# ViTAE-Transformer/MTP

Measured on AMD Instinct MI355X. Metric: images/sec pretrain step (ViT-L+RVSA, 224^2, bf16), higher is better.
Workload: dtype bf16; 1 GPU; ViT-L + RVSA backbone fwd+bwd + grad all-reduce + clip + AdamW, 224x224, batch 64 per GPU (BASELINE configs[2]/[3]); global_batch=64, parallelism=dp1, activation_checkpointing=False, heads=sum_i mean(f_i)

## Files before the change

### include/mtp_hip.h

```cpp
#ifndef MTP_HIP_H_
#define MTP_HIP_H_

#include <stddef.h>
#include <stdint.h>

#ifdef __cplusplus
extern "C" {
#endif

typedef void* mtp_stream_t;

typedef enum { MTP_F32 = 0, MTP_BF16 = 1, MTP_F64 = 2  } mtp_dtype;

enum { MTP_OK = 0, MTP_ERR_ARG = -1, MTP_ERR_UNSUPPORTED = -2 };

typedef enum {
    MTP_EPI_BIAS = 0,
    MTP_EPI_BIAS_GELU = 1,
    MTP_EPI_BIAS_RES = 2,
    MTP_EPI_DGELU = 3,
    MTP_EPI_BIAS_GELU_DG = 4,
    MTP_EPI_MUL = 5
} mtp_epilogue;

// ... 54 lines not shown

int mtp_gemm_nt(const mtp_gemm_args* args, mtp_stream_t stream);
typedef enum {
    MTP_GEMM_NT_FAMILY_SB = 0,
    MTP_GEMM_NT_FAMILY_SB8 = 1,
    MTP_GEMM_NT_FAMILY_REG = 2,
    MTP_GEMM_NT_FAMILY_P8 = 3,
    MTP_GEMM_NT_FAMILY_STRIP = 4
} mtp_gemm_nt_family;
struct mtp_gemm_nt_plan {
    int family;
    int tile_m;
    int order;
    int persistent;
    int store_policy;
};
int mtp_gemm_nt_plan(const mtp_gemm_args* args, int cus, struct mtp_gemm_nt_plan* out);
int mtp_gemm_nt_tile(const mtp_gemm_args* args);
int64_t mtp_gemm_nt_workspace_bytes(void);
int mtp_gemm_tn(const mtp_gemm_args* args, mtp_stream_t stream);
#define MTP_MAX_GROUPED_GEMMS 32
int mtp_gemm_tn_grouped(const mtp_gemm_args* args, int count, mtp_stream_t stream);
int mtp_sum_partials_batch(const float* const* parts, float* const* outs, const int64_t* numel, const int* splits, int count,
                           mtp_stream_t stream);

int mtp_layernorm_fwd(const void* x, int x_dtype, const float* gamma, const float* beta, void* y, int y_dtype,
                      float* mean, float* rstd, int64_t rows, int64_t C, float eps, int fuse_gelu, mtp_stream_t stream);
int64_t mtp_layernorm_bwd_partial_rows(int64_t rows);
int mtp_layernorm_bwd(const void* dy, int dy_dtype, const void* x, int x_dtype, const float* mean, const float* rstd,
                      const float* gamma, const float* beta, int fuse_gelu,
                      const float* dres, const float* extra, void* dx, int dx_dtype,
                      void* dx_copy, int copy_dtype, const float* copy_scale, int64_t rows_per_sample,
                      float* dgamma_part, float* dbeta_part, int64_t part_ld, int64_t rows, int64_t C, mtp_stream_t stream);
int mtp_layernorm_bwd_win(const void* dy, int dy_dtype, const void* x, int x_dtype, const float* mean, const float* rstd,
                          const float* gamma, const float* dres, const float* extra, void* dx, int dx_dtype,
                          void* dx_copy, int copy_dtype, const float* copy_scale, int64_t rows_per_sample,
                          float* dgamma_part, float* dbeta_part, int64_t part_ld, int64_t rows, int64_t C,
                          const float* win_add, int64_t B, int64_t Hp, int64_t Wp, mtp_stream_t stream);
int mtp_layernorm_residual_fwd(const void* h, int dtype, const float* gamma, const float* beta, const float* x, const float* layer_scale,
                               const float* sample_scale, int64_t rows_per_sample, float* out, void* out_act, float* mean, float* rstd,
                               int64_t rows, int64_t C, float eps, mtp_stream_t stream);
int mtp_layernorm_residual_bwd(const float* dout, const void* h, int dtype, const float* mean, const float* rstd, const float* gamma, const float* beta,
                               const float* layer_scale, const float* sample_scale, int64_t rows_per_sample, void* dh, float* part,
                               int64_t rows, int64_t C, mtp_stream_t stream);
int mtp_reduce_rows_f32(const float* part, int64_t ld, float* out, int64_t rows, int64_t C, int accumulate, mtp_stream_t stream);
#define MTP_REDUCE_BATCH_MAX 32
int mtp_reduce_rows_batched_f32(const float* const* parts, float* const* outs, int n, int64_t ld, int64_t rows, int64_t C, int accumulate,
                                mtp_stream_t stream);
int mtp_reduce_rows_t_f32(const float* part, int64_t ld, float* out, int64_t rows, int64_t R, int64_t C, int accumulate, mtp_stream_t stream);
int mtp_reduce_rows_t_batched_f32(const float* const* parts, float* const* outs, int n, int64_t ld, int64_t rows, int64_t R, int64_t C, int accumulate,
                                  mtp_stream_t stream);
int mtp_colsum(const void* dY, int dtype, int64_t ld, float* out, int64_t M, int64_t N, mtp_stream_t stream);
int mtp_colsum_acc(const void* dY, int dtype, int64_t ld, float* out, int64_t M, int64_t N, mtp_stream_t stream);

int mtp_patchify(const float* img, void* cols, int dtype, int64_t B, int64_t Cin, int64_t H, int64_t W, int64_t P, mtp_stream_t stream);
int mtp_unpatchify(const void* cols, int dtype, float* dimg, int64_t B, int64_t Cin, int64_t H, int64_t W, int64_t P, mtp_stream_t stream);
int mtp_preprocess_patchify(const uint8_t* img, void* cols, int dtype, int64_t B, int64_t H, int64_t W, int64_t P, int64_t pad_divisor,
                            const float* mean, const float* std, int bgr_to_rgb, float pad_value, mtp_stream_t stream);
int mtp_cast(const void* src, int src_dtype, void* dst, int dst_dtype, int64_t n, mtp_stream_t stream);
int mtp_transpose_cast(const float* src, void* dst, int dst_dtype, int64_t R, int64_t C, mtp_stream_t stream);
typedef struct {
    const float* src;
    void* w;
    void* wt;
    int64_t R, C;
    int64_t tile0;
    int32_t f32_out;
    float wd;
} mtp_wimg_desc;
int mtp_weight_images(const mtp_wimg_desc* descs_dev, int n, int64_t total_tiles, int act_dtype, mtp_stream_t stream);
int mtp_adamw_weight_images(const mtp_wimg_desc* descs_dev, int n, int64_t total_tiles, int act_dtype, float* p_base, const float* g_base, float* m_base, float* v_base,
                            const float* hyper, const float* sqnorm, float max_norm, float grad_scale, mtp_stream_t stream);
int mtp_adamw_weight_images_lr(const mtp_wimg_desc* descs_dev, const float* desc_lr, int n, int64_t total_tiles, int act_dtype, float* p_base, const float* g_base,
                               float* m_base, float* v_base, const float* hyper, const float* sqnorm, float max_norm, float grad_scale, mtp_stream_t stream);
int mtp_convt_pack(const float* w, void* wg, void* wgT, int dtype, int64_t Cin, int64_t Cout, mtp_stream_t stream);
int mtp_convt_unpack_grad(const float* dwg, float* dw, int64_t Cin, int64_t Cout, mtp_stream_t stream);
int mtp_tokens_to_nchw(const void* x, int x_dtype, void* out, int out_dtype, int64_t B, int64_t Hp, int64_t Wp, int64_t C, int levels, mtp_stream_t stream);
int mtp_nchw_to_tokens(const void* f, int f_dtype, void* out, int out_dtype, int64_t B, int64_t Hp, int64_t Wp, int64_t C, int levels, mtp_stream_t stream);
int mtp_maxpool2_tokens_fwd(const float* x, void* y, int y_dtype, int64_t B, int64_t Hp, int64_t Wp, int64_t C, mtp_stream_t stream);
int mtp_maxpool2_tokens_bwd(const float* x, const void* dy, int dy_dtype, float* dx, int accumulate, int64_t B, int64_t Hp, int64_t Wp, int64_t C, mtp_stream_t stream);
int mtp_axpy_f32(float* y, const float* x, float alpha, int64_t n, mtp_stream_t stream);
#define MTP_MAX_SEGMENTS 12
int mtp_copy_segments_f32(const float* const* src, float* const* dst, const int64_t* count, int n, mtp_stream_t stream);
int mtp_scale_rows_cast(const float* src, void* dst, int dst_dtype, const float* scale, int64_t rows_per_sample, int64_t rows, int64_t C, mtp_stream_t stream);

int mtp_im2col3x3(const void* x, int x_dtype, int64_t sN, int64_t sH, int64_t sW, int64_t sC, void* cols, int cols_dtype,
                  int64_t N, int64_t H, int64_t W, int64_t Cin, int64_t stride, int64_t Kp, mtp_stream_t stream);
int mtp_col2im3x3(const void* dcols, int cols_dtype, float* dx, int64_t sN, int64_t sH, int64_t sW, int64_t sC,
                  int64_t N, int64_t H, int64_t W, int64_t Cin, int64_t stride, int64_t Kp, int accumulate, mtp_stream_t stream);
int mtp_conv3x3_pack(const float* w, void* w2, void* w2t, int dtype, int64_t Cout, int64_t Cin, int64_t Kp, mtp_stream_t stream);
int mtp_conv3x3_unpack_grad(const float* dw2, float* dw, int64_t Cout, int64_t Cin, int64_t Kp, mtp_stream_t stream);
int mtp_pack_rows_padded(const float* w, void* wp, void* wpt, int dtype, int64_t R, int64_t C, int64_t Rp, mtp_stream_t stream);
int mtp_cast_pad_rows(const float* src, int64_t n, void* dst, int dst_dtype, int64_t ld, int64_t rows, mtp_stream_t stream);
int mtp_copy_rows(const void* src, int64_t src_ld, void* dst, int64_t dst_ld, int dtype, int64_t n, int64_t rows, mtp_stream_t stream);
int mtp_dwconv3x3_fwd(const void* x, const float* w, const float* bias, void* y, int dtype, int64_t N, int64_t H, int64_t W, int64_t C, mtp_stream_t stream);
int mtp_dwconv3x3_bwd_dx(const void* dy, int dtype, const float* w, float* dx, int accumulate, int64_t N, int64_t H, int64_t W, int64_t C, mtp_stream_t stream);
int64_t mtp_dwconv3x3_bwd_dw_partial_rows(int64_t N, int64_t H, int64_t W);
int mtp_dwconv3x3_bwd_dw(const void* dy, const void* x, int dtype, float* part, int64_t N, int64_t H, int64_t W, int64_t C, mtp_stream_t stream);
typedef enum { MTP_CONV_OP_IM2COL3X3 = 0, MTP_CONV_OP_COL2IM3X3 = 1, MTP_CONV_OP_DWCONV3X3_FWD = 2, MTP_CONV_OP_DWCONV3X3_BWD_DX = 3, MTP_CONV_OP_DWCONV3X3_BWD_DW = 4 } mtp_conv_op;
typedef enum {
    MTP_CONV_KERNEL_NONE = 0,
    MTP_CONV_KERNEL_ELEMENT = 1,
    MTP_CONV_KERNEL_V8 = 2,
    MTP_CONV_KERNEL_P8 = 3,
    MTP_CONV_KERNEL_PX4 = 4
} mtp_conv_kernel_family;
int mtp_conv_kernel(int op, const void* src, int src_dtype, int64_t sN, int64_t sH, int64_t sW, int64_t sC, const void* dst, int dst_dtype,
                    const float* w, const float* bias, int64_t N, int64_t H, int64_t W, int64_t C, int64_t stride, int64_t Kp);
int mtp_dwconv_fwd(const void* x, const float* w, const float* bias, void* y, int dtype, int64_t N, int64_t H, int64_t W, int64_t C, int k, mtp_stream_t stream);
int mtp_dwconv_bwd_dx(const void* dy, int dtype, const float* w, float* dx, int accumulate, int64_t N, int64_t H, int64_t W, int64_t C, int k, mtp_stream_t stream);
int mtp_dwconv_bwd_dw(const void* dy, const void* x, int dtype, float* dw, float* db, int64_t N, int64_t H, int64_t W, int64_t C, int k, mtp_stream_t stream);
// ... 24 lines not shown
    MTP_FULL_BWD_V3 = 1,
    MTP_FULL_BWD_FLASH = 3,
    MTP_FULL_BWD_THREE_PASS = 4,
    MTP_FULL_BWD_SINGLE_WG = 5,
    MTP_RVSA_FWD_GENERIC = 1,
    MTP_RVSA_FWD_MFMA = 2,
    MTP_RVSA_BWD_GENERIC = 1,
    MTP_RVSA_BWD_MFMA_DENSE = 2,
    MTP_RVSA_BWD_MFMA_ATOMIC = 3
};
int mtp_full_attn_kernel(int dtype, int64_t Hp, int64_t Wp, int backward);
int mtp_rvsa_attn_kernel(int dtype, int64_t Hp, int64_t Wp, int64_t heads, int backward);

int mtp_rvsa_pool_fwd(const void* x, int dtype, float* avg, float* pooled, int64_t B, int64_t Hp, int64_t Wp, int64_t C, mtp_stream_t stream);
int mtp_rvsa_pool_bwd(const float* dpooled, const float* avg, void* dx, int dtype, int accumulate, int64_t B, int64_t Hp, int64_t Wp, int64_t C, mtp_stream_t stream);
int mtp_rvsa_sampling_fwd(const void* x, int dtype, const float* w, const float* bias, float* avg, float* pooled, float* samp,
                          int64_t B, int64_t Hp, int64_t Wp, int64_t C, int64_t N, mtp_stream_t stream);
int mtp_rvsa_sampling_bwd(const float* dsamp, const float* w, const float* avg, void* dx, int dtype,
                          int64_t B, int64_t Hp, int64_t Wp, int64_t C, int64_t N, mtp_stream_t stream);
int mtp_rvsa_sampling_bwd_win(const float* dsamp, const float* w, const float* avg, float* g, int64_t windows, int64_t C, int64_t N, mtp_stream_t stream);
int mtp_small_linear_fwd(const float* x, const float* w, const float* b, float* y, int64_t R, int64_t N, int64_t K, mtp_stream_t stream);
int mtp_small_linear_bwd(const float* x, const float* w, const float* dy, float* dx, float* dw, float* db, int64_t R, int64_t N, int64_t K, mtp_stream_t stream);
int mtp_small_linear_dw_segments(const float* x, const float* dy, int64_t R, int64_t N, int64_t K, int nseg, const int64_t* seg_rows,
                                 float* const* dw, float* const* db, mtp_stream_t stream);
int mtp_small_linear_dw_segments_batched(const float* const* xs, const float* const* dys, int count, int64_t R, int64_t N, int64_t K, int nseg,
                                         const int64_t* seg_rows, float* const* dw, float* const* db, mtp_stream_t stream);
int mtp_rvsa_attn_fwd(const void* qkv, const float* samp, void* o, float* lse, int dtype,
                      const float* rel_h, const float* rel_w, const float* bias_table,
                      int64_t B, int64_t Hp, int64_t Wp, int64_t heads, int64_t hd, float scale, mtp_stream_t stream);
int mtp_rvsa_attn_bwd(const void* qkv, const float* samp, const void* o, const void* dout, const float* lse,
                      void* dqkv, float* dkv_f32, float* dsamp, float* rel_part, float* tab_part, int dtype,
                      const float* rel_h, const float* rel_w, const float* bias_table,
                      int64_t B, int64_t Hp, int64_t Wp, int64_t heads, int64_t hd, float scale, mtp_stream_t stream);

int mtp_zero_segments_f32(float* base, const int64_t* start, const int64_t* count, int n, mtp_stream_t stream);
int mtp_sqnorm_f32(const float* g, float* out, int64_t n, mtp_stream_t stream);
int mtp_sqnorm_segments_f32(const float* base, const int64_t* start, const int64_t* count, int n, float* out, mtp_stream_t stream);
int mtp_adamw_flat(float* p, const float* g, float* m, float* v, int64_t n, const int64_t* seg_start, const float* seg_wd, int nseg,
                   const float* hyper, const float* sqnorm, float max_norm, float grad_scale, mtp_stream_t stream);
int mtp_adamw_flat_lr(float* p, const float* g, float* m, float* v, int64_t n, const int64_t* seg_start, const float* seg_wd, const float* seg_lr, int nseg,
                      const float* hyper, const float* sqnorm, float max_norm, float grad_scale, mtp_stream_t stream);

typedef struct {
    int64_t N, H, W;
    int kernel_h, kernel_w, stride_h, stride_w, pad_h, pad_w, dilation_h, dilation_w;
    int group, group_channels;
    float offset_scale;
    int im2col_step;
    int remove_center;
    int variant;
} mtp_dcnv3_geom;
int mtp_dcnv3_out_size(const mtp_dcnv3_geom* geom, int64_t* Ho, int64_t* Wo);
int mtp_dcnv3_fwd(const void* input, const void* offset, const void* mask, void* output, int dtype, const mtp_dcnv3_geom* geom, mtp_stream_t stream);
int mtp_dcnv3_bwd(const void* input, const void* offset, const void* mask, const void* grad_output, int dtype, float* grad_input, float* grad_offset,
                  float* grad_mask, const mtp_dcnv3_geom* geom, mtp_stream_t stream);
int mtp_dcnv3_bwd_act(const void* input, const void* offset, const void* mask, const void* grad_output, int dtype, float* grad_input, float* grad_offset,
                      float* grad_mask, void* grad_offset_act, int64_t act_ld, const mtp_dcnv3_geom* geom, mtp_stream_t stream);

typedef enum {
    MTP_DCNV3_KERNEL_NONE = 0,
    MTP_DCNV3_FWD9 = 1,
    MTP_DCNV3_FWD_VEC8 = 2,
    MTP_DCNV3_FWD_SCALAR = 3,
    MTP_DCNV3_F64 = 4,
    MTP_DCNV3_BWD_WINDOW_R2 = 5,
    MTP_DCNV3_BWD_WINDOW_R3 = 6,
// ... 96 lines not shown
```

### mtp_amd/_lib.py

```python
import ctypes as C
import os

_HERE = os.path.dirname(os.path.abspath(__file__))
LIB_PATH = os.environ.get("MTP_HIP_LIB") or os.path.join(_HERE, "libmtp_hip.so")

MTP_F32, MTP_BF16, MTP_F64 = 0, 1, 2
EPI_BIAS, EPI_BIAS_GELU, EPI_BIAS_RES, EPI_DGELU, EPI_BIAS_GELU_DG, EPI_MUL = 0, 1, 2, 3, 4, 5

GEMM_NT_REG_STAGED = 1
GEMM_ORDER_SHIFT, GEMM_ORDER_PLAIN, GEMM_ORDER_GROUPED, GEMM_ORDER_ROW_MAJOR, GEMM_ORDER_MASK = 1, 1 << 1, 2 << 1, 3 << 1, 3 << 1
GEMM_TNG_PLAIN_ORDER = 1 << 1
GEMM_TN_REG_TRANSPOSE = 1 << 4
GEMM_NT_SB8, GEMM_NT_NO_SB8 = 1 << 5, 1 << 6
GEMM_NT_P8, GEMM_NT_P8_224, GEMM_NT_P8_256, GEMM_NT_P8_MASK, GEMM_NT_NO_P8 = 1 << 8, 2 << 8, 3 << 8, 3 << 8, 1 << 10
GEMM_NT_PERSIST, GEMM_TN_TR_FULL_ONLY, GEMM_NT_NO_PERSIST = 1 << 15, 1 << 15, 1 << 16
GEMM_NT_STRIP, GEMM_NT_NO_STRIP = 1 << 17, 1 << 18
GEMM_TNG_PLAIN_PHASES = 1 << 19
GEMM_STORE_SHIFT, GEMM_STORE_NT, GEMM_STORE_SC1, GEMM_STORE_PLAIN, GEMM_STORE_MASK = 20, 1 << 20, 2 << 20, 3 << 20, 3 << 20
GEMM_NT_FAMILY_SB, GEMM_NT_FAMILY_SB8, GEMM_NT_FAMILY_REG, GEMM_NT_FAMILY_P8, GEMM_NT_FAMILY_STRIP = 0, 1, 2, 3, 4

CONV_OP_IM2COL3X3, CONV_OP_COL2IM3X3, CONV_OP_DWCONV3X3_FWD, CONV_OP_DWCONV3X3_BWD_DX, CONV_OP_DWCONV3X3_BWD_DW = 0, 1, 2, 3, 4
CONV_KERNEL_NONE, CONV_KERNEL_ELEMENT, CONV_KERNEL_V8, CONV_KERNEL_P8, CONV_KERNEL_PX4 = 0, 1, 2, 3, 4
DCNV3_KERNEL_NONE, DCNV3_FWD9, DCNV3_FWD_VEC8, DCNV3_FWD_SCALAR, DCNV3_F64 = 0, 1, 2, 3, 4
DCNV3_BWD_WINDOW_R2, DCNV3_BWD_WINDOW_R3, DCNV3_BWD_3X3_OS1, DCNV3_BWD_3X3_OS2, DCNV3_BWD_SCATTER_SHFL, DCNV3_BWD_SCATTER_ATOMIC = 5, 6, 7, 8, 9, 10
# ... 23 lines not shown
class WimgDesc(C.Structure):
    _fields_ = [("src", p), ("w", p), ("wt", p), ("R", i64), ("C", i64), ("tile0", i64), ("f32_out", C.c_int32), ("wd", C.c_float)]


class Dcnv3Geom(C.Structure):
    _fields_ = [("N", i64), ("H", i64), ("W", i64), ("kernel_h", C.c_int32), ("kernel_w", C.c_int32), ("stride_h", C.c_int32), ("stride_w", C.c_int32),
                ("pad_h", C.c_int32), ("pad_w", C.c_int32), ("dilation_h", C.c_int32), ("dilation_w", C.c_int32), ("group", C.c_int32),
                ("group_channels", C.c_int32), ("offset_scale", C.c_float), ("im2col_step", C.c_int32), ("remove_center", C.c_int32), ("variant", C.c_int32)]


SIGNATURES = {
    "mtp_weight_images": (i32, [p, i32, i64, i32, p]),
    "mtp_dwconv_fwd": (i32, [p, p, p, p, i32, i64, i64, i64, i64, i32, p]),
    "mtp_dwconv_bwd_dx": (i32, [p, i32, p, p, i32, i64, i64, i64, i64, i32, p]),
    "mtp_dwconv_bwd_dw": (i32, [p, p, i32, p, p, i64, i64, i64, i64, i32, p]),
    "mtp_center_feature_scale_fwd": (i32, [p, p, p, i64, p, i32, i64, i64, i64, p]),
    "mtp_center_feature_scale_bwd": (i32, [p, p, p, p, i64, p, p, p, i32, i64, i64, i64, p]),
    "mtp_dcnv3_out_size": (i32, [C.POINTER(Dcnv3Geom), C.POINTER(i64), C.POINTER(i64)]),
    "mtp_dcnv3_fwd": (i32, [p, p, p, p, i32, C.POINTER(Dcnv3Geom), p]),
    "mtp_dcnv3_bwd": (i32, [p, p, p, p, i32, p, p, p, C.POINTER(Dcnv3Geom), p]),
    "mtp_dcnv3_bwd_act": (i32, [p, p, p, p, i32, p, p, p, p, i64, C.POINTER(Dcnv3Geom), p]),
    "mtp_dcnv3_kernel": (i32, [p, p, p, p, p, p, p, i32, C.POINTER(Dcnv3Geom), i32]),
    "mtp_conv_kernel": (i32, [i32, p, i32, i64, i64, i64, i64, p, i32, p, p, i64, i64, i64, i64, i64, i64]),
    "mtp_gemm_nt": (i32, [C.POINTER(GemmArgs), p]),
    "mtp_gemm_nt_plan": (i32, [C.POINTER(GemmArgs), i32, C.POINTER(GemmNtPlan)]),
    "mtp_gemm_nt_tile": (i32, [C.POINTER(GemmArgs)]),
    "mtp_gemm_nt_workspace_bytes": (i64, []),
    "mtp_gemm_tn": (i32, [C.POINTER(GemmArgs), p]),
    "mtp_gemm_tn_grouped": (i32, [C.POINTER(GemmArgs), i32, p]),
    "mtp_sum_partials_batch": (i32, [p, p, p, p, i32, p]),
    "mtp_layernorm_fwd": (i32, [p, i32, p, p, p, i32, p, p, i64, i64, f32, i32, p]),
    "mtp_layernorm_bwd_partial_rows": (i64, [i64]),
    "mtp_layernorm_bwd": (i32, [p, i32, p, i32, p, p, p, p, i32, p, p, p, i32, p, i32, p, i64, p, p, i64, i64, i64, p]),
    "mtp_reduce_rows_f32": (i32, [p, i64, p, i64, i64, i32, p]),
    "mtp_reduce_rows_batched_f32": (i32, [p, p, i32, i64, i64, i64, i32, p]),
    "mtp_reduce_rows_t_f32": (i32, [p, i64, p, i64, i64, i64, i32, p]),
    "mtp_reduce_rows_t_batched_f32": (i32, [p, p, i32, i64, i64, i64, i64, i32, p]),
    "mtp_copy_segments_f32": (i32, [p, p, p, i32, p]),
    "mtp_colsum": (i32, [p, i32, i64, p, i64, i64, p]),
    "mtp_colsum_acc": (i32, [p, i32, i64, p, i64, i64, p]),
    "mtp_patchify": (i32, [p, p, i32, i64, i64, i64, i64, i64, p]),
    "mtp_preprocess_patchify": (i32, [p, p, i32, i64, i64, i64, i64, i64, C.POINTER(f32), C.POINTER(f32), i32, f32, p]),
    "mtp_unpatchify": (i32, [p, i32, p, i64, i64, i64, i64, i64, p]),
    "mtp_cast": (i32, [p, i32, p, i32, i64, p]),
    "mtp_transpose_cast": (i32, [p, p, i32, i64, i64, p]),
    "mtp_convt_pack": (i32, [p, p, p, i32, i64, i64, p]),
    "mtp_convt_unpack_grad": (i32, [p, p, i64, i64, p]),
    "mtp_tokens_to_nchw": (i32, [p, i32, p, i32, i64, i64, i64, i64, i32, p]),
    "mtp_nchw_to_tokens": (i32, [p, i32, p, i32, i64, i64, i64, i64, i32, p]),
    "mtp_maxpool2_tokens_fwd": (i32, [p, p, i32, i64, i64, i64, i64, p]),
    "mtp_maxpool2_tokens_bwd": (i32, [p, p, i32, p, i32, i64, i64, i64, i64, p]),
    "mtp_axpy_f32": (i32, [p, p, f32, i64, p]),
    "mtp_scale_rows_cast": (i32, [p, p, i32, p, i64, i64, i64, p]),
    "mtp_im2col3x3": (i32, [p, i32, i64, i64, i64, i64, p, i32, i64, i64, i64, i64, i64, i64, p]),
    "mtp_col2im3x3": (i32, [p, i32, p, i64, i64, i64, i64, i64, i64, i64, i64, i64, i64, i32, p]),
    "mtp_conv3x3_pack": (i32, [p, p, p, i32, i64, i64, i64, p]),
    "mtp_conv3x3_unpack_grad": (i32, [p, p, i64, i64, i64, p]),
    "mtp_pack_rows_padded": (i32, [p, p, p, i32, i64, i64, i64, p]),
    "mtp_cast_pad_rows": (i32, [p, i64, p, i32, i64, i64, p]),
    "mtp_copy_rows": (i32, [p, i64, p, i64, i32, i64, i64, p]),
    "mtp_dwconv3x3_fwd": (i32, [p, p, p, p, i32, i64, i64, i64, i64, p]),
    "mtp_dwconv3x3_bwd_dx": (i32, [p, i32, p, p, i32, i64, i64, i64, i64, p]),
    "mtp_dwconv3x3_bwd_dw_partial_rows": (i64, [i64, i64, i64]),
    "mtp_dwconv3x3_bwd_dw": (i32, [p, p, i32, p, i64, i64, i64, i64, p]),
    "mtp_softmax_groups_fwd": (i32, [p, i64, p, i32, i64, i64, i64, p]),
    "mtp_softmax_groups_bwd": (i32, [p, p, p, i64, i32, i64, i64, i64, p]),
    "mtp_scale_residual_fwd": (i32, [p, p, i32, p, p, i64, p, p, i64, i64, p]),
    "mtp_scale_residual_bwd_partial_rows": (i64, [i64]),
    "mtp_scale_residual_bwd": (i32, [p, p, i32, p, p, i64, p, p, i64, i64, p]),
    "mtp_comm_unique_id": (i32, [p]),
    "mtp_comm_init": (i32, [p, i32, i32, C.POINTER(C.c_void_p)]),
    "mtp_comm_allreduce_bucket": (i32, [p, p, i64, p]),
    "mtp_comm_allreduce_bucket_dt": (i32, [p, p, i64, i32, p]),
    "mtp_comm_reduce_scatter_bucket": (i32, [p, p, i64, i32, i32, p]),
    "mtp_comm_allgather_bucket": (i32, [p, p, i64, i32, i32, p]),
    "mtp_comm_info": (i32, [p, p]),
    "mtp_comm_destroy": (i32, [p]),
    "mtp_full_attn_fwd": (i32, [p, p, p, i32, p, p, i64, i64, i64, i64, i64, f32, p]),
    "mtp_full_attn_bwd_workspace_floats": (i64, [i64, i64, i64, i64]),
    "mtp_full_attn_bwd": (i32, [p, p, p, p, p, i32, p, p, p, p, i64, i64, i64, i64, i64, f32, p]),
    "mtp_full_attn_kernel": (i32, [i32, i64, i64, i32]),
    "mtp_rvsa_attn_kernel": (i32, [i32, i64, i64, i64, i32]),
    "mtp_rvsa_pool_fwd": (i32, [p, i32, p, p, i64, i64, i64, i64, p]),
    "mtp_rvsa_pool_bwd": (i32, [p, p, p, i32, i32, i64, i64, i64, i64, p]),
    "mtp_rvsa_sampling_fwd": (i32, [p, i32, p, p, p, p, p, i64, i64, i64, i64, i64, p]),
    "mtp_rvsa_sampling_bwd": (i32, [p, p, p, p, i32, i64, i64, i64, i64, i64, p]),
    "mtp_rvsa_sampling_bwd_win": (i32, [p, p, p, p, i64, i64, i64, p]),
    "mtp_layernorm_residual_fwd": (i32, [p, i32, p, p, p, p, p, i64, p, p, p, p, i64, i64, f32, p]),
    "mtp_layernorm_residual_bwd": (i32, [p, p, i32, p, p, p, p, p, p, i64, p, p, i64, i64, p]),
    "mtp_layernorm_bwd_win": (i32, [p, i32, p, i32, p, p, p, p, p, p, i32, p, i32, p, i64, p, p, i64, i64, i64, p, i64, i64, i64, p]),
    "mtp_small_linear_fwd": (i32, [p, p, p, p, i64, i64, i64, p]),
    "mtp_small_linear_bwd": (i32, [p, p, p, p, p, p, i64, i64, i64, p]),
    "mtp_small_linear_dw_segments": (i32, [p, p, i64, i64, i64, i32, p, p, p, p]),
    "mtp_small_linear_dw_segments_batched": (i32, [p, p, i32, i64, i64, i64, i32, p, p, p, p]),
    "mtp_rvsa_attn_fwd": (i32, [p, p, p, p, i32, p, p, p, i64, i64, i64, i64, i64, f32, p]),
    "mtp_rvsa_attn_bwd": (i32, [p, p, p, p, p, p, p, p, p, p, i32, p, p, p, i64, i64, i64, i64, i64, f32, p]),
    "mtp_zero_segments_f32": (i32, [p, p, p, i32, p]),
    "mtp_sqnorm_f32": (i32, [p, p, i64, p]),
    "mtp_sqnorm_segments_f32": (i32, [p, p, p, i32, p, p]),
    "mtp_adamw_flat": (i32, [p, p, p, p, i64, p, p, i32, p, p, f32, f32, p]),
    "mtp_adamw_weight_images": (i32, [p, i32, i64, i32, p, p, p, p, p, p, f32, f32, p]),
    "mtp_adamw_flat_lr": (i32, [p, p, p, p, i64, p, p, p, i32, p, p, f32, f32, p]),
    "mtp_adamw_weight_images_lr": (i32, [p, p, i32, i64, i32, p, p, p, p, p, p, f32, f32, p]),
    "mtp_bn_partial_rows": (i64, [i64]),
    "mtp_bn_stats": (i32, [p, i32, i64, p, p, p, i64, i64, p]),
    "mtp_bn_finalize": (i32, [p, p, C.c_double, p, p, f32, f32, p, p, i64, p]),
    "mtp_bn_apply": (i32, [p, i32, i64, p, p, p, p, i32, p, i32, i64, i64, i64, p]),
    "mtp_bn_bwd_stats": (i32, [p, i32, i64, p, i32, i64, p, p, p, p, i32, p, p, i64, i64, p]),
    "mtp_bn_bwd_dx": (i32, [p, i32, i64, p, i32, i64, p, p, p, p, i32, p, C.c_double, p, i32, i64, i64, i64, p]),
    "mtp_resize_bilinear_fwd": (i32, [p, i32, i64, p, i32, i64, i64, i64, i64, i64, i64, i64, i32, p]),
    "mtp_resize_bilinear_bwd": (i32, [p, i32, i64, p, i64, i64, i64, i64, i64, i64, i64, i32, p]),
    "mtp_adaptive_avg_pool_fwd": (i32, [p, i32, i64, p, i32, i64, i64, i64, i64, i64, p]),
    "mtp_adaptive_avg_pool_bwd": (i32, [p, i32, p, i64, i64, i64, i64, i64, i64, i32, p]),
    "mtp_channel_scale": (i32, [p, i32, i64, p, i64, p, i32, i64, i64, i64, p]),
    "mtp_seg_ce_workspace_bytes": (i64, [i64, i64, i64, i64]),
    "mtp_seg_ce": (i32, [p, i32, i64, i64, i64, i64, i64, p, i32, i64, i64, i32, f32, p, p, i64, p, i64, p]),
    "mtp_seg_window_accumulate": (i32, [p, i32, i64, i64, i64, i64, i64, p, i64, i64, i64, i64, i64, i64, i64, p]),
    "mtp_seg_argmax_areas": (i32, [p, i64, i64, i64, i64, i64, p, p, i32, p, p, p, i32, i32, p, p]),
    "mtp_seg_areas": (i32, [p, i32, p, i32, i64, i64, i32, p, p]),
    "mtp_fuse_pair_fwd": (i32, [p, i32, p, i32, i64, i64, i64, i64, i64, i32, p]),
    "mtp_fuse_pair_bwd": (i32, [p, i64, p, i32, p, i64, i64, i64, i64, i32, p]),
    "mtp_unet_up_cat_fwd": (i32, [p, i64, i64, p, i64, i64, i32, p, i32, i64, i64, i64, i64, i64, i64, p]),
    "mtp_unet_up_cat_bwd": (i32, [p, i64, p, i64, i64, p, i64, i64, i64, i64, i64, i64, i64, i32, p]),
    "mtp_gap_fwd": (i32, [p, i32, p, i64, i64, i64, p]),
    "mtp_gap_bwd": (i32, [p, p, i32, i64, i64, i64, p]),
    "mtp_cls_ce": (i32, [p, p, p, p, f32, p, p, p, p, p, p, p, i64, i64, i64, p]),
    "mtp_cls_head_bwd": (i32, [p, p, p, p, p, p, i64, i64, i64, i32, p]),
    "mtp_cls_hits": (i32, [p, p, i64, i64, C.POINTER(C.c_int32), i32, f32, i32, p, p]),
    "mtp_box_iou": (i32, [p, p, p, i64, i64, i32, i32, i32, f32, p]),
# ... 41 lines not shown
```

### mtp_amd/csrc/attn.hip

```cpp
#include <stdlib.h>

#include "attn_launch.h"
#include "attn_rvsa_common.h"

namespace {

constexpr int KT = 32;

template <typename T>
__device__ __forceinline__ void load_row(const T* p, float (&r)[HD], float mul = 1.0f) {
#pragma unroll
    for (int i = 0; i < HD / 8; ++i) {
        float t[8];
        load8(p + 8 * i, t);
#pragma unroll
        for (int e = 0; e < 8; ++e) r[8 * i + e] = t[e] * mul;
    }
}
template <typename T>
__device__ __forceinline__ void store_row(T* p, const float (&r)[HD], float mul = 1.0f) {
#pragma unroll
    for (int i = 0; i < HD / 8; ++i) {
        float t[8];
#pragma unroll
// ... 799 lines not shown
                               (const float*)workspace, N, (int)Hp, (int)Wp, (int)heads, scale);
        }
        return mtp_launch_status();
    }
    const size_t lds = full_bwd1_lds(Hp, Wp);
    dim3 grid((unsigned)(B * heads)), block(256);
    hipStream_t s = (hipStream_t)stream;
    if (dtype == MTP_BF16) {
        (void)hipFuncSetAttribute((const void*)full_attn_bwd_kernel<bf16_t>, hipFuncAttributeMaxDynamicSharedMemorySize, (int)lds);
        hipLaunchKernelGGL((full_attn_bwd_kernel<bf16_t>), grid, block, lds, s, (const bf16_t*)qkv, (const bf16_t*)o, (const bf16_t*)dout, lse, (bf16_t*)dqkv,
                           rel_h, rel_w, drel_part, N, (int)Hp, (int)Wp, (int)heads, scale);
    } else {
        (void)hipFuncSetAttribute((const void*)full_attn_bwd_kernel<float>, hipFuncAttributeMaxDynamicSharedMemorySize, (int)lds);
        hipLaunchKernelGGL((full_attn_bwd_kernel<float>), grid, block, lds, s, (const float*)qkv, (const float*)o, (const float*)dout, lse, (float*)dqkv,
                           rel_h, rel_w, drel_part, N, (int)Hp, (int)Wp, (int)heads, scale);
    }
    return mtp_launch_status();
}

extern "C" int mtp_rvsa_attn_fwd(const void* qkv, const float* samp, void* o, float* lse, int dtype,
                                 const float* rel_h, const float* rel_w, const float* bias_table,
                                 int64_t B, int64_t Hp, int64_t Wp, int64_t heads, int64_t hd, float scale, mtp_stream_t stream) {
    if (!qkv || !samp || !o || !lse || !rel_h || !rel_w || !bias_table || B <= 0 || Hp < 7 || Wp < 7 || heads <= 0) return MTP_ERR_ARG;
    if (hd != HD) return MTP_ERR_UNSUPPORTED;
    const RvsaGeom g = make_geom(Hp, Wp, heads);
    dim3 grid((unsigned)(B * g.nh * g.nw * heads)), block(64);
    hipStream_t s = (hipStream_t)stream;
    if (rvsa_fwd_family(dtype) == MTP_RVSA_FWD_MFMA)
        return mtp_rvsa_fwd_mfma_launch(qkv, samp, o, lse, rel_h, rel_w, bias_table, B, Hp, Wp, heads, scale, s);
    hipLaunchKernelGGL(rvsa_attn_fwd_kernel, grid, block, 0, s, (const float*)qkv, samp, (float*)o, lse, rel_h, rel_w, bias_table, g, scale);
    return mtp_launch_status();
}

extern "C" int mtp_rvsa_attn_bwd(const void* qkv, const float* samp, const void* o, const void* dout, const float* lse,
                                 void* dqkv, float* dkv_f32, float* dsamp, float* rel_part, float* tab_part, int dtype,
                                 const float* rel_h, const float* rel_w, const float* bias_table,
                                 int64_t B, int64_t Hp, int64_t Wp, int64_t heads, int64_t hd, float scale, mtp_stream_t stream) {
    if (!qkv || !samp || !o || !dout || !lse || !dqkv || !dkv_f32 || !dsamp || !rel_part || !tab_part || !rel_h || !rel_w || !bias_table) return MTP_ERR_ARG;
    if (B <= 0 || Hp < 7 || Wp < 7 || heads <= 0) return MTP_ERR_ARG;
    if (hd != HD) return MTP_ERR_UNSUPPORTED;
    const RvsaGeom g = make_geom(Hp, Wp, heads);
    const int64_t Ttok = B * Hp * Wp, C = heads * HD;
    hipStream_t s = (hipStream_t)stream;
    const int family = rvsa_bwd_family(dtype, Hp, Wp, heads);
    if (family == MTP_RVSA_BWD_MFMA_DENSE)
        return mtp_rvsa_bwd_mfma_launch(qkv, samp, o, dout, lse, dqkv, dkv_f32, dsamp, rel_part, tab_part, rel_h, rel_w, bias_table, B, Hp, Wp, heads, scale, s);
    hipError_t e = hipMemsetAsync(dkv_f32, 0, sizeof(float) * (size_t)(Ttok * 2 * C), s);
    if (e != hipSuccess) return (int)e;
    dim3 grid((unsigned)(B * g.nh * g.nw * heads)), block(64);
    int64_t cb = (Ttok * 2 * C / 4 + 255) / 256;
    dim3 cgrid((unsigned)(cb > 8192 ? 8192 : cb)), cblock(256);
    if (family == MTP_RVSA_BWD_MFMA_ATOMIC) {
        const int rc = mtp_rvsa_bwd_mfma_launch(qkv, samp, o, dout, lse, dqkv, dkv_f32, dsamp, rel_part, tab_part, rel_h, rel_w, bias_table, B, Hp, Wp, heads, scale, s);
        if (rc) return rc;
        hipLaunchKernelGGL((dkv_convert_kernel<bf16_t>), cgrid, cblock, 0, s, dkv_f32, (bf16_t*)dqkv, Ttok, (int)C);
    } else {
        hipLaunchKernelGGL(rvsa_attn_bwd_kernel, grid, block, 0, s, (const float*)qkv, samp, (const float*)o, (const float*)dout, lse, (float*)dqkv,
                           dkv_f32, dsamp, rel_part, tab_part, rel_h, rel_w, bias_table, g, scale);
        hipLaunchKernelGGL((dkv_convert_kernel<float>), cgrid, cblock, 0, s, dkv_f32, (float*)dqkv, Ttok, (int)C);
    }
    return mtp_launch_status();
}
```

### mtp_amd/csrc/attn_launch.h

```cpp
#pragma once
#include <hip/hip_runtime.h>
#include <stdint.h>

int mtp_rvsa_fwd_mfma_launch(const void* qkv, const float* samp, void* o, float* lse, const float* rel_h, const float* rel_w, const float* bias_table,
                             int64_t B, int64_t Hp, int64_t Wp, int64_t heads, float scale, hipStream_t s);
int mtp_rvsa_bwd_mfma_launch(const void* qkv, const float* samp, const void* o, const void* dout, const float* lse, void* dqkv, float* dkv, float* dsamp,
                             float* rel_part, float* tab_part, const float* rel_h, const float* rel_w, const float* bias_table,
                             int64_t B, int64_t Hp, int64_t Wp, int64_t heads, float scale, hipStream_t s);
int mtp_rvsa_bwd_mfma_scatter_mode(int64_t Hp, int64_t Wp, int64_t heads);
bool mtp_full_v3_fits(int64_t Hp, int64_t Wp);
int mtp_full_fwd_flash_keys(int64_t Hp, int64_t Wp);
bool mtp_full_bwd_flash_fits(int64_t Hp, int64_t Wp);
int mtp_full_v3_fwd_launch(const void* qkv, void* o, float* lse, const float* rel_h, const float* rel_w, int64_t B, int64_t Hp, int64_t Wp, int64_t heads,
                           float scale, hipStream_t s);
int mtp_full_v3_bwd_launch(const void* qkv, const void* o, const void* dout, const float* lse, void* dqkv, const float* rel_h, const float* rel_w,
                           float* drel_part, int64_t B, int64_t Hp, int64_t Wp, int64_t heads, float scale, hipStream_t s);
int mtp_full_fwd_flash_launch(const void* qkv, void* o, float* lse, const float* rel_h, const float* rel_w, int64_t B, int64_t Hp, int64_t Wp, int64_t heads,
                              float scale, hipStream_t s);
int mtp_full_bwd_flash_launch(const void* qkv, const void* o, const void* dout, const float* lse, void* dqkv, const float* rel_h, const float* rel_w,
                              float* drel_part, float* workspace, int64_t B, int64_t Hp, int64_t Wp, int64_t heads, float scale, hipStream_t s);
```

### mtp_amd/csrc/attn_rvsa_bwd4.hip

```cpp
#include <stdlib.h>

#include "attn_launch.h"
#include "attn_rvsa_common.h"

namespace {

typedef __attribute__((ext_vector_type(2))) __bf16 bf16x2v_t;
constexpr int TP = 136;
constexpr int SMP_F = 18;

__global__ __launch_bounds__(256, 3) void rvsa_bwd5_mfma_kernel(const bf16_t* __restrict__ qkv, const float* __restrict__ samp, const bf16_t* __restrict__ o, const bf16_t* __restrict__ dout,
                                                            const float* __restrict__ lse, bf16_t* __restrict__ dqkv, float* __restrict__ dkv, float* __restrict__ dsamp,
                                                            float* __restrict__ rel_part, float* __restrict__ tab_part,
                                                            const float* __restrict__ rel_h, const float* __restrict__ rel_w, const float* __restrict__ bias_table,
                                                            RvsaGeom g, float scale) {
    __shared__ __attribute__((aligned(16))) char Ks[64 * 128];
    __shared__ __attribute__((aligned(16))) char Vs[64 * 128];
    __shared__ __attribute__((aligned(16))) char R2[2 * 64 * 128];
    __shared__ float QR[26 * 64];
    constexpr int DQP = 65;
    __shared__ float dQR[26 * DQP];
    __shared__ float tab[176];
    __shared__ float lses[64];
    __shared__ float delta[64];
// ... 784 lines not shown
#pragma unroll
            for (int kk = 0; kk < 2; ++kk) {
                float w[8];
#pragma unroll
                for (int e = 0; e < 8; ++e)
                    w[e] = live * fmaxf(0.f, 1.f - fabsf(kx[8 * kk + e] - X)) * fmaxf(0.f, 1.f - fabsf(ky[8 * kk + e] - Y));
                af[kk] = pack_bf16x8(w[0], w[1], w[2], w[3], w[4], w[5], w[6], w[7]);
            }
#pragma unroll
            for (int dt = 0; dt < 4; ++dt) {
                f32x4_t ak = {0.f, 0.f, 0.f, 0.f}, av = {0.f, 0.f, 0.f, 0.f};
#pragma unroll
                for (int kk = 0; kk < 2; ++kk) {
                    ak = mma(af[kk], bk[dt][kk], ak);
                    av = mma(af[kk], bv[dt][kk], av);
                }
#pragma unroll
                for (int r = 0; r < 4; ++r) {
                    const int t2 = 16 * ti + 4 * gq + r;
                    if (t2 < N) {
                        float* drow = dkv + ((int64_t)b * N + t2) * (2 * C) + h * HD + 16 * dt + fr;
                        if (ak[r] != 0.f) atomicAdd(drow, ak[r]);
                        if (av[r] != 0.f) atomicAdd(drow + C, av[r]);
                    }
                }
            }
        }
    }
}

constexpr int SCB = 224;

__global__ __launch_bounds__(256, 2) void rvsa_scatter_gemm_kernel(const bf16_t* __restrict__ dsel, const float* __restrict__ samp, bf16_t* __restrict__ dqkv,
                                                                  RvsaGeom g) {
    __shared__ __attribute__((aligned(16))) char Kimg[SCB * 128];
    __shared__ __attribute__((aligned(16))) char Vimg[SCB * 128];
    __shared__ __attribute__((aligned(16))) float xs[SCB];
    __shared__ __attribute__((aligned(16))) float ys[SCB];
    const int tid = threadIdx.x, lane = tid & 63, wave = tid >> 6, fr = lane & 15, gq = lane >> 4;
    const int H = g.heads, nW = g.nh * g.nw, S = nW * 49;
    const int h = blockIdx.x % H, b = blockIdx.x / H;
    const int C = H * HD, N = g.Hp * g.Wp;
    const int t0 = blockIdx.y * SCB, nt = (N - t0) < SCB ? (N - t0) : SCB;
    const int64_t ld = 3 * (int64_t)C;
    float X[4], Y[4], live[4];
    f32x4_t dk[4][4], dv[4][4];
#pragma unroll
    for (int i = 0; i < 4; ++i) {
        const int tl = 16 * (wave + 4 * i) + fr;
        const int tc = t0 + (tl < nt ? tl : nt - 1);
        const int ty = tc / g.Wp, tx = tc - ty * g.Wp;
        X[i] = (float)(tx + g.pad_l);
        Y[i] = (float)(ty + g.pad_t);
        live[i] = tl < nt ? 1.f : 0.f;
#pragma unroll
        for (int dt = 0; dt < 4; ++dt) {
            dk[i][dt] = f32x4_t{0.f, 0.f, 0.f, 0.f};
            dv[i][dt] = f32x4_t{0.f, 0.f, 0.f, 0.f};
        }
    }
    const int ntile = (nt + 15) / 16;
    const float ylo = (float)(t0 / g.Wp + g.pad_t) - 1.0f, yhi = (float)((t0 + nt - 1) / g.Wp + g.pad_t) + 1.0f;
    for (int c0 = 0; c0 < S; c0 += SCB) {
        __syncthreads();
        int hit = 0;
        if (tid < SCB) {
            const int sg = c0 + tid;
            float x = -1.0e4f, y = -1.0e4f;
            if (sg < S) {
                const int w = sg / 49, k = sg - 49 * w;
                const Sample sa = make_sample<true>(g, samp + (int64_t)(b * nW + w) * 5 * H, h, w / g.nw, w % g.nw, k / 7, k % 7);
                x = (float)sa.x0 + sa.fx;
                y = (float)sa.y0 + sa.fy;
            }
// ... 57 lines not shown
#pragma unroll
    for (int i = 0; i < 4; ++i) {
        const int tl = 16 * (wave + 4 * i) + fr;
        if (tl < nt) {
#pragma unroll
            for (int dt = 0; dt < 4; ++dt) {
                const int o = tl * 128 + (((2 * dt + (gq >> 1)) ^ (tl & 7)) << 4) + (gq & 1) * 8;
                *reinterpret_cast<uint2*>(Kimg + o) = make_uint2(pack_bf16x2(dk[i][dt][0], dk[i][dt][1]), pack_bf16x2(dk[i][dt][2], dk[i][dt][3]));
                *reinterpret_cast<uint2*>(Vimg + o) = make_uint2(pack_bf16x2(dv[i][dt][0], dv[i][dt][1]), pack_bf16x2(dv[i][dt][2], dv[i][dt][3]));
            }
        }
    }
    __syncthreads();
    for (int idx = tid; idx < nt * 16; idx += 256) {
        const int tl = idx >> 4, m = (idx >> 3) & 1, ch = idx & 7;
        const uint4 v = *reinterpret_cast<const uint4*>((m ? Vimg : Kimg) + swz(tl, ch));
        *reinterpret_cast<uint4*>(dqkv + ((int64_t)b * N + t0 + tl) * ld + (1 + m) * C + h * HD + 8 * ch) = v;
    }
}

}

int mtp_rvsa_bwd_mfma_scatter_mode(int64_t Hp, int64_t Wp, int64_t heads) {
    static const bool dense = []() { const char* e = getenv("MTP_RVSA_SCATTER"); return e && e[0] == 'd'; }();
    if (dense) return 1;
    const RvsaGeom g = make_geom(Hp, Wp, heads);
    const int64_t N = Hp * Wp, nW = (int64_t)g.nh * g.nw;
    const bool fits = Hp <= 64 && Wp <= 64 && nW * (2 * 49 * HD * 2) <= N * 2 * HD * 4;
    return fits ? 4 : 1;
}

int mtp_rvsa_bwd_mfma_launch(const void* qkv, const float* samp, const void* o, const void* dout, const float* lse, void* dqkv, float* dkv, float* dsamp,
                             float* rel_part, float* tab_part, const float* rel_h, const float* rel_w, const float* bias_table,
                             int64_t B, int64_t Hp, int64_t Wp, int64_t heads, float scale, hipStream_t s) {
    const RvsaGeom g = make_geom(Hp, Wp, heads);
    const int mode = mtp_rvsa_bwd_mfma_scatter_mode(Hp, Wp, heads);
    const dim3 grid((unsigned)(B * g.nh * g.nw * heads));
    if (mode == 4) {
        static const bool old4 = []() { const char* e = getenv("MTP_RVSA_BWD"); return e && e[0] == '4'; }();
        if (old4)
            hipLaunchKernelGGL(rvsa_bwd4_mfma_kernel<4>, grid, dim3(256), 0, s, (const bf16_t*)qkv, samp, (const bf16_t*)o, (const bf16_t*)dout, lse,
                               (bf16_t*)dqkv, dkv, dsamp, rel_part, tab_part, rel_h, rel_w, bias_table, g, scale);
        else
            hipLaunchKernelGGL(rvsa_bwd5_mfma_kernel, grid, dim3(256), 0, s, (const bf16_t*)qkv, samp, (const bf16_t*)o, (const bf16_t*)dout, lse,
                               (bf16_t*)dqkv, dkv, dsamp, rel_part, tab_part, rel_h, rel_w, bias_table, g, scale);
        const int64_t N = Hp * Wp;
        hipLaunchKernelGGL(rvsa_scatter_gemm_kernel, dim3((unsigned)(B * heads), (unsigned)((N + SCB - 1) / SCB)), dim3(256), 0, s, (const bf16_t*)dkv, samp, (bf16_t*)dqkv, g);
    } else {
        hipLaunchKernelGGL(rvsa_bwd4_mfma_kernel<1>, grid, dim3(256), 0, s, (const bf16_t*)qkv, samp, (const bf16_t*)o, (const bf16_t*)dout, lse,
                           (bf16_t*)dqkv, dkv, dsamp, rel_part, tab_part, rel_h, rel_w, bias_table, g, scale);
    }
    return mtp_launch_status();
}
```

### mtp_amd/csrc/common.h

```cpp
#pragma once
#include <hip/hip_runtime.h>
#include <stdint.h>

#include "../../include/mtp_hip.h"

#define MTP_WAVE 64

typedef __attribute__((ext_vector_type(8))) __bf16 bf16x8_t;
typedef __attribute__((ext_vector_type(4))) float f32x4_t;

struct bf16_t {
    uint16_t bits;
};

__device__ __forceinline__ float bf16_bits_to_f32(uint32_t b) { return __uint_as_float(b << 16); }
__device__ __forceinline__ uint32_t f32_to_bf16_bits(float f) {
    uint32_t u = __float_as_uint(f);
    if ((u & 0x7fffffffu) > 0x7f800000u) return (u >> 16) | 0x40u;
    return (u + 0x7fffu + ((u >> 16) & 1u)) >> 16;
}
typedef __attribute__((ext_vector_type(2))) __bf16 bf16x2_t;
typedef __attribute__((ext_vector_type(2))) float f32x2_t;
__device__ __forceinline__ uint32_t pack_bf16x2(float lo, float hi) {
    f32x2_t v = {lo, hi};
// ... 102 lines not shown
    else if constexpr (M == 2) return dpp_mov<0x4E>(v);
    else if constexpr (M == 4) return dpp_mov<0x1B>(dpp_mov<0x141>(v));
    else return dpp_mov<0x141>(dpp_mov<0x140>(v));
}
__device__ __forceinline__ float xor16_sum(float v) {
    const auto r = __builtin_amdgcn_permlane16_swap(__float_as_uint(v), __float_as_uint(v), false, false);
    return __uint_as_float(r[0]) + __uint_as_float(r[1]);
}
__device__ __forceinline__ float xor32_sum(float v) {
    const auto r = __builtin_amdgcn_permlane32_swap(__float_as_uint(v), __float_as_uint(v), false, false);
    return __uint_as_float(r[0]) + __uint_as_float(r[1]);
}
__device__ __forceinline__ float xor16_max(float v) {
    const auto r = __builtin_amdgcn_permlane16_swap(__float_as_uint(v), __float_as_uint(v), false, false);
    return fmaxf(__uint_as_float(r[0]), __uint_as_float(r[1]));
}
__device__ __forceinline__ float xor32_max(float v) {
    const auto r = __builtin_amdgcn_permlane32_swap(__float_as_uint(v), __float_as_uint(v), false, false);
    return fmaxf(__uint_as_float(r[0]), __uint_as_float(r[1]));
}
__device__ __forceinline__ float rows_sum(float v) { return xor32_sum(xor16_sum(v)); }
__device__ __forceinline__ float rows_max(float v) { return xor32_max(xor16_max(v)); }
__device__ __forceinline__ float wave_sum(float v) {
    v = xor32_sum(v); v = xor16_sum(v);
    v += lane_xor<8>(v); v += lane_xor<4>(v); v += lane_xor<2>(v); v += lane_xor<1>(v);
    return v;
}
__device__ __forceinline__ float wave_max(float v) {
    v = xor32_max(v); v = xor16_max(v);
    v = fmaxf(v, lane_xor<8>(v)); v = fmaxf(v, lane_xor<4>(v)); v = fmaxf(v, lane_xor<2>(v)); v = fmaxf(v, lane_xor<1>(v));
    return v;
}

static inline int mtp_optin_lds(const void* kern, int bytes, unsigned long long& mask) {
    int dev = 0;
    if (hipGetDevice(&dev) != hipSuccess) dev = 64;
    if (dev < 64 && ((mask >> dev) & 1ull)) return 0;
    const hipError_t e = hipFuncSetAttribute(kern, hipFuncAttributeMaxDynamicSharedMemorySize, bytes);
    if (e != hipSuccess) return (int)e;
    if (dev < 64) mask |= 1ull << dev;
    return 0;
}

#define MTP_CHECK_ARG(cond) \
    do {                    \
        if (!(cond)) return MTP_ERR_ARG; \
    } while (0)

int mtp_stream_cus(hipStream_t stream);

static inline int mtp_launch_status() {
    hipError_t e = hipGetLastError();
    return e == hipSuccess ? 0 : (int)e;
}
```

### mtp_amd/csrc/elementwise.hip

```cpp
#include "common.h"
#include <atomic>
#include <mutex>

namespace {

inline unsigned blocks_for(int64_t n, int per_block, int64_t cap = 1 << 20) {
    int64_t b = (n + per_block - 1) / per_block;
    return (unsigned)(b < 1 ? 1 : (b > cap ? cap : b));
}

template <typename T, bool INVERSE>
__global__ __launch_bounds__(256) void patchify_kernel(float* __restrict__ img, T* __restrict__ cols, int B, int Cin, int H, int W, int P, int Hp, int Wp) {
    const int K4 = Cin * P * P / 4, P4 = P / 4;
    const int64_t total = (int64_t)B * Hp * Wp * K4;
    for (int64_t i = (int64_t)blockIdx.x * 256 + threadIdx.x; i < total; i += (int64_t)gridDim.x * 256) {
        const int k4 = (int)(i % K4);
        const int64_t t = i / K4;
        const int kx4 = k4 % P4, ky = (k4 / P4) % P, c = k4 / (P4 * P);
        const int px = (int)(t % Wp), py = (int)((t / Wp) % Hp), b = (int)(t / ((int64_t)Wp * Hp));
        float* ip = img + (((int64_t)b * Cin + c) * H + py * P + ky) * W + px * P + kx4 * 4;
        T* cp = cols + t * (K4 * 4) + k4 * 4;
        if (INVERSE)
            *reinterpret_cast<float4*>(ip) = load4(cp);
        else
            store4(cp, *reinterpret_cast<const float4*>(ip));
    }
}

template <typename Ts, typename Td>
__global__ __launch_bounds__(256) void cast_kernel(const Ts* __restrict__ s, Td* __restrict__ d, int64_t n) {
    const int64_t n4 = n >> 2;
    for (int64_t i = (int64_t)blockIdx.x * 256 + threadIdx.x; i < n4; i += (int64_t)gridDim.x * 256) store4(d + 4 * i, load4(s + 4 * i));
    if (blockIdx.x == 0 && threadIdx.x < (n & 3)) Elem<Td>::store(d + (n4 << 2) + threadIdx.x, Elem<Ts>::load(s + (n4 << 2) + threadIdx.x));
}

__device__ __forceinline__ int64_t pixel_to_row(int64_t s, int Wp, int L) {
    if (L == 0) return s;
    const int Wo = Wp << L;
    const int y = (int)(s / Wo), x = (int)(s % Wo);
    int64_t r = (int64_t)(y >> L) * Wp + (x >> L);
    for (int l = 1; l <= L; ++l) r = r * 4 + (((y >> (L - l)) & 1) << 1) + ((x >> (L - l)) & 1);
    return r;
}

template <typename Tin, typename Tout, bool ROWS2COLS>
__global__ __launch_bounds__(256) void transpose_kernel(const Tin* __restrict__ in, Tout* __restrict__ out, int64_t S, int64_t C, int Wp, int L) {
    __shared__ float tile[64][65];
    const int64_t bt = blockIdx.z;
    const int64_t s0 = (int64_t)blockIdx.x * 64, c0 = (int64_t)blockIdx.y * 64;
    const Tin* ib = in + bt * S * C;
    Tout* ob = out + bt * S * C;
    const int t = threadIdx.x;
    const int a = t >> 2, g = (t & 3) * 16;
    if (ROWS2COLS) {
        const int64_t s = s0 + a;
        if (s < S) {
            const Tin* rp = ib + pixel_to_row(s, Wp, L) * C + c0 + g;
#pragma unroll
            for (int v = 0; v < 4; ++v) {
                if (c0 + g + 4 * v < C) {
                    const float4 x = load4(rp + 4 * v);
                    tile[g + 4 * v + 0][a] = x.x; tile[g + 4 * v + 1][a] = x.y; tile[g + 4 * v + 2][a] = x.z; tile[g + 4 * v + 3][a] = x.w;
                }
            }
        }
        __syncthreads();
        const int64_t c = c0 + a;
        if (c < C) {
            Tout* wp = ob + c * S + s0 + g;
#pragma unroll
            for (int v = 0; v < 4; ++v) {
                const int64_t s2 = s0 + g + 4 * v;
                if (s2 + 3 < S && (S & 3) == 0) {
                    store4(wp + 4 * v, make_float4(tile[a][g + 4 * v], tile[a][g + 4 * v + 1], tile[a][g + 4 * v + 2], tile[a][g + 4 * v + 3]));
                } else {
                    for (int e = 0; e < 4; ++e)
                        if (s2 + e < S) Elem<Tout>::store(wp + 4 * v + e, tile[a][g + 4 * v + e]);
                }
            }
        }
    } else {
        const int64_t c = c0 + a;
        if (c < C) {
            const Tin* rp = ib + c * S + s0 + g;
#pragma unroll
            for (int v = 0; v < 4; ++v) {
                const int64_t s2 = s0 + g + 4 * v;
                if (s2 + 3 < S && (S & 3) == 0) {
                    const float4 x = load4(rp + 4 * v);
                    tile[a][g + 4 * v] = x.x; tile[a][g + 4 * v + 1] = x.y; tile[a][g + 4 * v + 2] = x.z; tile[a][g + 4 * v + 3] = x.w;
                } else {
                    for (int e = 0; e < 4; ++e)
                        if (s2 + e < S) tile[a][g + 4 * v + e] = Elem<Tin>::load(rp + 4 * v + e);
                }
            }
        }
        __syncthreads();
        const int64_t s = s0 + a;
        if (s < S) {
            Tout* wp = ob + pixel_to_row(s, Wp, L) * C + c0 + g;
#pragma unroll
            for (int v = 0; v < 4; ++v)
                if (c0 + g + 4 * v < C)
                    store4(wp + 4 * v, make_float4(tile[g + 4 * v][a], tile[g + 4 * v + 1][a], tile[g + 4 * v + 2][a], tile[g + 4 * v + 3][a]));
        }
    }
}

template <bool ROWS2COLS>
__global__ __launch_bounds__(256) void transpose8_bf16_kernel(const bf16_t* __restrict__ in, bf16_t* __restrict__ out, int64_t S, int64_t C, int Wp, int L) {
    __shared__ float tile[64][65];
    const int64_t bt = blockIdx.z;
    const int64_t s0 = (int64_t)blockIdx.x * 64, c0 = (int64_t)blockIdx.y * 64;
    const bf16_t* ib = in + bt * S * C;
    bf16_t* ob = out + bt * S * C;
    const int t = threadIdx.x, ra = t >> 3, cg = (t & 7) * 8;
    float x[8];
    if (ROWS2COLS) {
#pragma unroll
        for (int h = 0; h < 2; ++h) {
            const int64_t sp = s0 + ra + 32 * h;
            if (sp < S && c0 + cg < C) {
                load8(ib + pixel_to_row(sp, Wp, L) * C + c0 + cg, x);
#pragma unroll
                for (int e = 0; e < 8; ++e) tile[cg + e][ra + 32 * h] = x[e];
            }
        }
        __syncthreads();
#pragma unroll
        for (int h = 0; h < 2; ++h) {
            const int64_t c = c0 + ra + 32 * h;
            if (c < C && s0 + cg < S) {
#pragma unroll
                for (int e = 0; e < 8; ++e) x[e] = tile[ra + 32 * h][cg + e];
                store8(ob + c * S + s0 + cg, x);
            }
        }
    } else {
#pragma unroll
        for (int h = 0; h < 2; ++h) {
            const int64_t c = c0 + ra + 32 * h;
            if (c < C && s0 + cg < S) {
                load8(ib + c * S + s0 + cg, x);
#pragma unroll
                for (int e = 0; e < 8; ++e) tile[ra + 32 * h][cg + e] = x[e];
            }
        }
        __syncthreads();
#pragma unroll
        for (int h = 0; h < 2; ++h) {
            const int64_t sp = s0 + ra + 32 * h;
            if (sp < S && c0 + cg < C) {
#pragma unroll
                for (int e = 0; e < 8; ++e) x[e] = tile[cg + e][ra + 32 * h];
                store8(ob + pixel_to_row(sp, Wp, L) * C + c0 + cg, x);
            }
        }
    }
}

template <bool ROWS2COLS>
int launch_transpose(const void* in, int in_dt, void* out, int out_dt, int64_t batches, int64_t S, int64_t C, int Wp, int L, hipStream_t s) {
    if (C % 4) return MTP_ERR_ARG;
    dim3 grid((unsigned)((S + 63) / 64), (unsigned)((C + 63) / 64), (unsigned)batches), block(256);
    if (in_dt == MTP_BF16 && out_dt == MTP_BF16 && !(S & 7) && !(C & 7) && !(((uintptr_t)in | (uintptr_t)out) & 15)) {
        hipLaunchKernelGGL((transpose8_bf16_kernel<ROWS2COLS>), grid, block, 0, s, (const bf16_t*)in, (bf16_t*)out, S, C, Wp, L);
        return mtp_launch_status();
    }
#define MTP_TR(TI, TO) hipLaunchKernelGGL((transpose_kernel<TI, TO, ROWS2COLS>), grid, block, 0, s, (const TI*)in, (TO*)out, S, C, Wp, L)
    if (in_dt == MTP_F32 && out_dt == MTP_F32) MTP_TR(float, float);
    else if (in_dt == MTP_F32 && out_dt == MTP_BF16) MTP_TR(float, bf16_t);
    else if (in_dt == MTP_BF16 && out_dt == MTP_F32) MTP_TR(bf16_t, float);
    else if (in_dt == MTP_BF16 && out_dt == MTP_BF16) MTP_TR(bf16_t, bf16_t);
    else return MTP_ERR_UNSUPPORTED;
#undef MTP_TR
    return mtp_launch_status();
}

template <typename T>
__global__ __launch_bounds__(256) void convt_pack_kernel(const float* __restrict__ w, T* __restrict__ wg, T* __restrict__ wgT, int64_t Cin, int64_t Cout) {
    const int64_t total = Cin * Cout * 4;
    for (int64_t i = (int64_t)blockIdx.x * 256 + threadIdx.x; i < total; i += (int64_t)gridDim.x * 256) {
        const int q = (int)(i & 3);
        const int64_t co = (i >> 2) % Cout, ci = (i >> 2) / Cout;
        const float v = w[i];
        if (wg) Elem<T>::store(wg + (q * Cout + co) * Cin + ci, v);
        if (wgT) Elem<T>::store(wgT + ci * (4 * Cout) + q * Cout + co, v);
    }
}
__global__ __launch_bounds__(256) void convt_unpack_kernel(const float* __restrict__ dwg, float* __restrict__ dw, int64_t Cin, int64_t Cout) {
    const int64_t total = Cin * Cout * 4;
    for (int64_t i = (int64_t)blockIdx.x * 256 + threadIdx.x; i < total; i += (int64_t)gridDim.x * 256) {
        const int q = (int)(i & 3);
        const int64_t co = (i >> 2) % Cout, ci = (i >> 2) / Cout;
        dw[i] = dwg[(q * Cout + co) * Cin + ci];
    }
}

template <typename T>
__global__ __launch_bounds__(256) void convt_pack_tiled_kernel(const float* __restrict__ w, T* __restrict__ wg, T* __restrict__ wgT, int Cin, int Cout) {
    __shared__ float tile[2][64][65];
    const int ci0 = blockIdx.y * 64, co0 = blockIdx.x * 64;
// ... 749 lines not shown
        if (dtype == MTP_BF16)
            hipLaunchKernelGGL((convt_pack_tiled_kernel<bf16_t>), tg, dim3(256), 0, (hipStream_t)stream, w, (bf16_t*)wg, (bf16_t*)wgT, (int)Cin, (int)Cout);
        else
            hipLaunchKernelGGL((convt_pack_tiled_kernel<float>), tg, dim3(256), 0, (hipStream_t)stream, w, (float*)wg, (float*)wgT, (int)Cin, (int)Cout);
        return mtp_launch_status();
    }
    dim3 grid(blocks_for(Cin * Cout * 4, 256, 4096)), block(256);
    if (dtype == MTP_BF16)
        hipLaunchKernelGGL((convt_pack_kernel<bf16_t>), grid, block, 0, (hipStream_t)stream, w, (bf16_t*)wg, (bf16_t*)wgT, Cin, Cout);
    else
        hipLaunchKernelGGL((convt_pack_kernel<float>), grid, block, 0, (hipStream_t)stream, w, (float*)wg, (float*)wgT, Cin, Cout);
    return mtp_launch_status();
}

extern "C" int mtp_convt_unpack_grad(const float* dwg, float* dw, int64_t Cin, int64_t Cout, mtp_stream_t stream) {
    if (!dwg || !dw || Cin <= 0 || Cout <= 0) return MTP_ERR_ARG;
    if (!(Cin & 7) && !(Cout & 7) && Cin < (1 << 20) && Cout < (1 << 20)) {
        hipLaunchKernelGGL(convt_unpack_tiled_kernel, dim3((unsigned)((Cout + 63) / 64), (unsigned)((Cin + 63) / 64)), dim3(256), 0, (hipStream_t)stream, dwg, dw, (int)Cin, (int)Cout);
        return mtp_launch_status();
    }
    hipLaunchKernelGGL(convt_unpack_kernel, dim3(blocks_for(Cin * Cout * 4, 256, 4096)), dim3(256), 0, (hipStream_t)stream, dwg, dw, Cin, Cout);
    return mtp_launch_status();
}

extern "C" int mtp_tokens_to_nchw(const void* x, int x_dtype, void* out, int out_dtype, int64_t B, int64_t Hp, int64_t Wp, int64_t C, int levels, mtp_stream_t stream) {
    if (!x || !out || B <= 0 || Hp <= 0 || Wp <= 0 || levels < 0 || levels > 4) return MTP_ERR_ARG;
    return launch_transpose<true>(x, x_dtype, out, out_dtype, B, (Hp * Wp) << (2 * levels), C, (int)Wp, levels, (hipStream_t)stream);
}
extern "C" int mtp_nchw_to_tokens(const void* f, int f_dtype, void* out, int out_dtype, int64_t B, int64_t Hp, int64_t Wp, int64_t C, int levels, mtp_stream_t stream) {
    if (!f || !out || B <= 0 || Hp <= 0 || Wp <= 0 || levels < 0 || levels > 4) return MTP_ERR_ARG;
    return launch_transpose<false>(f, f_dtype, out, out_dtype, B, (Hp * Wp) << (2 * levels), C, (int)Wp, levels, (hipStream_t)stream);
}

extern "C" int mtp_maxpool2_tokens_fwd(const float* x, void* y, int y_dtype, int64_t B, int64_t Hp, int64_t Wp, int64_t C, mtp_stream_t stream) {
    if (!x || !y || B <= 0 || Hp < 2 || Wp < 2 || (C % 4)) return MTP_ERR_ARG;
    dim3 grid(blocks_for(B * (Hp / 2) * (Wp / 2) * C / 4, 256, 8192)), block(256);
    if (y_dtype == MTP_BF16)
        hipLaunchKernelGGL((maxpool_fwd_kernel<bf16_t>), grid, block, 0, (hipStream_t)stream, x, (bf16_t*)y, (int)B, (int)Hp, (int)Wp, (int)C);
    else
        hipLaunchKernelGGL((maxpool_fwd_kernel<float>), grid, block, 0, (hipStream_t)stream, x, (float*)y, (int)B, (int)Hp, (int)Wp, (int)C);
    return mtp_launch_status();
}
extern "C" int mtp_maxpool2_tokens_bwd(const float* x, const void* dy, int dy_dtype, float* dx, int accumulate, int64_t B, int64_t Hp, int64_t Wp, int64_t C, mtp_stream_t stream) {
    if (!x || !dy || !dx || B <= 0 || Hp < 2 || Wp < 2 || (C % 4)) return MTP_ERR_ARG;
    dim3 grid(blocks_for(B * Hp * Wp * C / 4, 256, 8192)), block(256);
    if (dy_dtype == MTP_BF16)
        hipLaunchKernelGGL((maxpool_bwd_kernel<bf16_t>), grid, block, 0, (hipStream_t)stream, x, (const bf16_t*)dy, dx, accumulate, (int)B, (int)Hp, (int)Wp, (int)C);
    else
        hipLaunchKernelGGL((maxpool_bwd_kernel<float>), grid, block, 0, (hipStream_t)stream, x, (const float*)dy, dx, accumulate, (int)B, (int)Hp, (int)Wp, (int)C);
    return mtp_launch_status();
}

extern "C" int mtp_axpy_f32(float* y, const float* x, float alpha, int64_t n, mtp_stream_t stream) {
    if (!y || !x || n <= 0) return MTP_ERR_ARG;
    hipLaunchKernelGGL(axpy_kernel, dim3(blocks_for(n, 256, 8192)), dim3(256), 0, (hipStream_t)stream, y, x, alpha, n);
    return mtp_launch_status();
}

struct CopySegs {
    const float* src[MTP_MAX_SEGMENTS];
    float* dst[MTP_MAX_SEGMENTS];
    int64_t count[MTP_MAX_SEGMENTS];
};
__global__ __launch_bounds__(256) void copy_segments_kernel(CopySegs t) {
    const int sgm = blockIdx.y;
    const float* __restrict__ s = t.src[sgm];
// ... 109 lines not shown
        }
    }
    part[q][lane] = d;
    __syncthreads();
    if (!live) return;
    const float4 p0 = part[0][lane], p1 = part[1][lane], p2 = part[2][lane], p3 = part[3][lane];
    d = make_float4((p0.x + p1.x) + (p2.x + p3.x), (p0.y + p1.y) + (p2.y + p3.y), (p0.z + p1.z) + (p2.z + p3.z), (p0.w + p1.w) + (p2.w + p3.w));
    const float4 a = load4(avg + (int64_t)win * C + 4 * c4);
    const float k = 1.0f / 49.0f;
    const float4 g = make_float4(d.x * (a.x > 0 ? k : 0.01f * k), d.y * (a.y > 0 ? k : 0.01f * k), d.z * (a.z > 0 ? k : 0.01f * k), d.w * (a.w > 0 ? k : 0.01f * k));
#pragma unroll 1
    for (int aa = q; aa < 7; aa += 4) {
        const int y = i * 7 + aa - pad_t;
        if (y < 0 || y >= Hp) continue;
        float4 o[7];
#pragma unroll
        for (int bb = 0; bb < 7; ++bb) {
            const int xx = j * 7 + bb - pad_l;
            const int xc = (xx >= 0 && xx < Wp) ? xx : 0;
            o[bb] = load4(dx + (((int64_t)b * Hp + y) * Wp + xc) * C + 4 * c4);
        }
#pragma unroll
        for (int bb = 0; bb < 7; ++bb) {
            const int xx = j * 7 + bb - pad_l;
            if (xx >= 0 && xx < Wp)
                store4(dx + (((int64_t)b * Hp + y) * Wp + xx) * C + 4 * c4, make_float4(o[bb].x + g.x, o[bb].y + g.y, o[bb].z + g.z, o[bb].w + g.w));
        }
    }
}

__global__ __launch_bounds__(256) void rvsa_sampling_bwd_win_kernel(const float* __restrict__ dsamp, const float* __restrict__ w, const float* __restrict__ avg,
                                                                   float* __restrict__ g, int C, int N) {
    extern __shared__ __attribute__((aligned(16))) float ds[];
    __shared__ float4 part[4][64];
    const int win = blockIdx.x;
    const int lane = threadIdx.x & 63, q = threadIdx.x >> 6;
    const int c4 = blockIdx.y * 64 + lane;
    const bool live = c4 < C / 4;
    for (int n = threadIdx.x; n < N; n += 256) ds[n] = dsamp[(int64_t)win * N + n];
    __syncthreads();
    const int nq = (N + 3) / 4, n0 = q * nq, n1 = (n0 + nq) < N ? (n0 + nq) : N;
    float4 d = make_float4(0, 0, 0, 0);
    if (live) {
#pragma unroll 10
        for (int n = n0; n < n1; ++n) {
            const float4 ww = load4(w + (int64_t)n * C + 4 * c4);
            const float t = ds[n];
            d.x += t * ww.x; d.y += t * ww.y; d.z += t * ww.z; d.w += t * ww.w;
        }
    }
    part[q][lane] = d;
    __syncthreads();
    if (!live || q) return;
    const float4 p0 = part[0][lane], p1 = part[1][lane], p2 = part[2][lane], p3 = part[3][lane];
    d = make_float4((p0.x + p1.x) + (p2.x + p3.x), (p0.y + p1.y) + (p2.y + p3.y), (p0.z + p1.z) + (p2.z + p3.z), (p0.w + p1.w) + (p2.w + p3.w));
    const float4 a = load4(avg + (int64_t)win * C + 4 * c4);
    const float k = 1.0f / 49.0f;
    *reinterpret_cast<float4*>(g + (int64_t)win * C + 4 * c4) =
        make_float4(d.x * (a.x > 0 ? k : 0.01f * k), d.y * (a.y > 0 ? k : 0.01f * k), d.z * (a.z > 0 ? k : 0.01f * k), d.w * (a.w > 0 ? k : 0.01f * k));
}

extern "C" int mtp_rvsa_sampling_bwd_win(const float* dsamp, const float* w, const float* avg, float* g, int64_t windows, int64_t C, int64_t N, mtp_stream_t stream) {
    if (!dsamp || !w || !avg || !g || windows <= 0 || C <= 0 || (C % 4) || N <= 0 || N > 4096) return MTP_ERR_ARG;
    const dim3 grid((unsigned)windows, (unsigned)((C / 4 + 63) / 64)), block(256);
    hipLaunchKernelGGL(rvsa_sampling_bwd_win_kernel, grid, block, sizeof(float) * (size_t)N, (hipStream_t)stream, dsamp, w, avg, g, (int)C, (int)N);
    return mtp_launch_status();
}

extern "C" int mtp_rvsa_sampling_fwd(const void* x, int dtype, const float* w, const float* bias, float* avg, float* pooled, float* samp,
                                     int64_t B, int64_t Hp, int64_t Wp, int64_t C, int64_t N, mtp_stream_t stream) {
    if (!x || !w || !avg || !pooled || !samp || B <= 0 || Hp <= 0 || Wp <= 0 || C <= 0 || (C % 4) || C > 8192 || N <= 0) return MTP_ERR_ARG;
    int pt, pl, nh, nw;
    rvsa_geom(Hp, Wp, pt, pl, nh, nw);
    constexpr int ysplit = 2;
    const dim3 grid((unsigned)(B * nh * nw), (unsigned)(N >= 16 * ysplit ? ysplit : 1)), block(256);
    const size_t lds = sizeof(float) * (size_t)C;
    if (dtype == MTP_BF16)
        hipLaunchKernelGGL((rvsa_sampling_fwd_kernel<bf16_t>), grid, block, lds, (hipStream_t)stream, (const bf16_t*)x, w, bias, avg, pooled, samp, (int)Hp, (int)Wp, (int)C, (int)N, pt, pl, nh, nw);
    else if (dtype == MTP_F32)
        hipLaunchKernelGGL((rvsa_sampling_fwd_kernel<float>), grid, block, lds, (hipStream_t)stream, (const float*)x, w, bias, avg, pooled, samp, (int)Hp, (int)Wp, (int)C, (int)N, pt, pl, nh, nw);
    else return MTP_ERR_UNSUPPORTED;
    return mtp_launch_status();
}
extern "C" int mtp_rvsa_sampling_bwd(const float* dsamp, const float* w, const float* avg, void* dx, int dtype,
                                     int64_t B, int64_t Hp, int64_t Wp, int64_t C, int64_t N, mtp_stream_t stream) {
    if (!dsamp || !w || !avg || !dx || B <= 0 || Hp <= 0 || Wp <= 0 || C <= 0 || (C % 4) || N <= 0 || N > 4096) return MTP_ERR_ARG;
    int pt, pl, nh, nw;
    rvsa_geom(Hp, Wp, pt, pl, nh, nw);
    const dim3 grid((unsigned)(B * nh * nw), (unsigned)((C / 4 + 63) / 64)), block(256);
    const size_t lds = sizeof(float) * (size_t)N;
    if (dtype == MTP_BF16)
        hipLaunchKernelGGL((rvsa_sampling_bwd_kernel<bf16_t>), grid, block, lds, (hipStream_t)stream, dsamp, w, avg, (bf16_t*)dx, (int)Hp, (int)Wp, (int)C, (int)N, pt, pl, nh, nw);
// ... 279 lines not shown
```

### mtp_amd/csrc/layernorm.hip

```cpp
#include "common.h"

namespace {

constexpr int LN_THREADS = 256;
constexpr int MAXV = 8;

template <typename Tx, typename Ty, bool GELU, int MV>
__global__ __launch_bounds__(LN_THREADS) void ln_fwd_kernel(const Tx* __restrict__ x, const float* __restrict__ gamma, const float* __restrict__ beta,
                                                           Ty* __restrict__ y, float* __restrict__ mean, float* __restrict__ rstd,
                                                           int64_t rows, int C, float eps) {
    const int lane = threadIdx.x & 63, wave = threadIdx.x >> 6;
    const int nv = C >> 2;
    int col[MV];
    bool ok[MV];
    float4 g[MV], bb[MV];
#pragma unroll
    for (int i = 0; i < MV; ++i) {
        const int c4 = lane + 64 * i;
        ok[i] = c4 < nv;
        col[i] = 4 * (ok[i] ? c4 : nv - 1);
        g[i] = *reinterpret_cast<const float4*>(gamma + col[i]);
        bb[i] = *reinterpret_cast<const float4*>(beta + col[i]);
    }
    for (int64_t row = (int64_t)blockIdx.x * 4 + wave; row < rows; row += (int64_t)gridDim.x * 4) {
        const Tx* xr = x + row * C;
        float4 v[MV];
#pragma unroll
        for (int i = 0; i < MV; ++i) v[i] = load4(xr + col[i]);
        float s = 0.f;
#pragma unroll
        for (int i = 0; i < MV; ++i) s += ok[i] ? (v[i].x + v[i].y + v[i].z + v[i].w) : 0.f;
        const float mu = wave_sum(s) / (float)C;
        float q = 0.f;
#pragma unroll
        for (int i = 0; i < MV; ++i) {
            const float a = v[i].x - mu, b = v[i].y - mu, c = v[i].z - mu, d = v[i].w - mu;
            q += ok[i] ? (a * a + b * b + c * c + d * d) : 0.f;
        }
        const float rs = rsqrtf(wave_sum(q) / (float)C + eps);
        if (lane == 0) {
            if (mean) mean[row] = mu;
            if (rstd) rstd[row] = rs;
        }
        Ty* yr = y + row * C;
#pragma unroll
        for (int i = 0; i < MV; ++i) {
            float4 o = make_float4((v[i].x - mu) * rs * g[i].x + bb[i].x, (v[i].y - mu) * rs * g[i].y + bb[i].y,
                                   (v[i].z - mu) * rs * g[i].z + bb[i].z, (v[i].w - mu) * rs * g[i].w + bb[i].w);
            if (GELU) o = make_float4(gelu_f(o.x), gelu_f(o.y), gelu_f(o.z), gelu_f(o.w));
            if (ok[i]) store4(yr + col[i], o);
        }
    }
}

struct LnWin { int Hp, Wp, pad_t, pad_l, nh, nw; };

template <typename Tact, typename Tx, typename Tdx, bool GELU, int MV>
__global__ __launch_bounds__(LN_THREADS) void ln_bwd_kernel(const Tact* __restrict__ dy, const Tx* __restrict__ x, const float* __restrict__ mean,
                                                           const float* __restrict__ rstd, const float* __restrict__ gamma, const float* __restrict__ beta,
                                                           const float* __restrict__ dres, const float* __restrict__ extra, Tdx* __restrict__ dx,
                                                           Tact* __restrict__ dx_copy, const float* __restrict__ copy_scale, int rows_per_sample,
                                                           float* __restrict__ dgamma_part, float* __restrict__ dbeta_part, int64_t part_ld, int64_t rows, int C,
                                                           const float* __restrict__ win_add, LnWin wg) {
    __shared__ float4 red[2][3][64 * MV];
    const int lane = threadIdx.x & 63, wave = threadIdx.x >> 6;
    const int nv = C >> 2;
    float4 gacc[MV], bacc[MV], g[MV], bt[MV];
    int col[MV];
    bool ok[MV];
#pragma unroll
    for (int i = 0; i < MV; ++i) {
        gacc[i] = make_float4(0, 0, 0, 0);
        bacc[i] = make_float4(0, 0, 0, 0);
        const int c4 = lane + 64 * i;
        ok[i] = c4 < nv;
        col[i] = 4 * (ok[i] ? c4 : nv - 1);
        g[i] = *reinterpret_cast<const float4*>(gamma + col[i]);
        bt[i] = GELU ? *reinterpret_cast<const float4*>(beta + col[i]) : make_float4(0, 0, 0, 0);
    }
    const float4 zero4 = make_float4(0.f, 0.f, 0.f, 0.f);
    for (int64_t row = (int64_t)blockIdx.x * 4 + wave; row < rows; row += (int64_t)gridDim.x * 4) {
        float4 xv[MV], dv[MV], rr[MV], ee[MV];
#pragma unroll
        for (int i = 0; i < MV; ++i) {
            xv[i] = load4(x + row * C + col[i]);
            dv[i] = load4(dy + row * C + col[i]);
            rr[i] = zero4;
            ee[i] = zero4;
        }
        if (dres) {
#pragma unroll
            for (int i = 0; i < MV; ++i) rr[i] = *reinterpret_cast<const float4*>(dres + row * C + col[i]);
        }
        if (extra) {
#pragma unroll
            for (int i = 0; i < MV; ++i) ee[i] = *reinterpret_cast<const float4*>(extra + row * C + col[i]);
        }
        float4 wa[MV];
#pragma unroll
        for (int i = 0; i < MV; ++i) wa[i] = zero4;
// ... 3 lines not shown
            const uint32_t win = (b * (uint32_t)wg.nh + (y + (uint32_t)wg.pad_t) / 7u) * (uint32_t)wg.nw + (xq + (uint32_t)wg.pad_l) / 7u;
            const float* wrow = win_add + (int64_t)win * C;
#pragma unroll
            for (int i = 0; i < MV; ++i) wa[i] = *reinterpret_cast<const float4*>(wrow + col[i]);
        }
        const float mu = mean[row], rs = rstd[row];
        const float cs = (dx_copy && copy_scale) ? copy_scale[(uint32_t)row / (uint32_t)rows_per_sample] : 1.0f;
        float4 xh[MV], d[MV];
        float s1 = 0.f, s2 = 0.f;
#pragma unroll
        for (int i = 0; i < MV; ++i) {
            dv[i].x += wa[i].x; dv[i].y += wa[i].y; dv[i].z += wa[i].z; dv[i].w += wa[i].w;
            if (!ok[i]) dv[i] = zero4;
            xh[i] = make_float4((xv[i].x - mu) * rs, (xv[i].y - mu) * rs, (xv[i].z - mu) * rs, (xv[i].w - mu) * rs);
            if (GELU) {
                dv[i].x *= dgelu_f(xh[i].x * g[i].x + bt[i].x);
                dv[i].y *= dgelu_f(xh[i].y * g[i].y + bt[i].y);
                dv[i].z *= dgelu_f(xh[i].z * g[i].z + bt[i].z);
                dv[i].w *= dgelu_f(xh[i].w * g[i].w + bt[i].w);
            }
            gacc[i].x += dv[i].x * xh[i].x; gacc[i].y += dv[i].y * xh[i].y; gacc[i].z += dv[i].z * xh[i].z; gacc[i].w += dv[i].w * xh[i].w;
            bacc[i].x += dv[i].x; bacc[i].y += dv[i].y; bacc[i].z += dv[i].z; bacc[i].w += dv[i].w;
            d[i] = make_float4(dv[i].x * g[i].x, dv[i].y * g[i].y, dv[i].z * g[i].z, dv[i].w * g[i].w);
            s1 += d[i].x * xh[i].x + d[i].y * xh[i].y + d[i].z * xh[i].z + d[i].w * xh[i].w;
            s2 += d[i].x + d[i].y + d[i].z + d[i].w;
        }
        const float c1 = wave_sum(s1) / (float)C, c2 = wave_sum(s2) / (float)C;
#pragma unroll
        for (int i = 0; i < MV; ++i) {
            const float4 o = make_float4((d[i].x - xh[i].x * c1 - c2) * rs + rr[i].x + ee[i].x, (d[i].y - xh[i].y * c1 - c2) * rs + rr[i].y + ee[i].y,
                                         (d[i].z - xh[i].z * c1 - c2) * rs + rr[i].z + ee[i].z, (d[i].w - xh[i].w * c1 - c2) * rs + rr[i].w + ee[i].w);
            if (ok[i]) {
                store4(dx + row * C + col[i], o);
                if (dx_copy) store4(dx_copy + row * C + col[i], make_float4(o.x * cs, o.y * cs, o.z * cs, o.w * cs));
            }
        }
    }
    if (wave > 0) {
#pragma unroll
        for (int i = 0; i < MV; ++i) {
            red[0][wave - 1][lane + 64 * i] = gacc[i];
            red[1][wave - 1][lane + 64 * i] = bacc[i];
        }
    }
    __syncthreads();
    if (wave == 0) {
#pragma unroll
        for (int i = 0; i < MV; ++i) {
            if (ok[i]) {
                float4 a = gacc[i], b = bacc[i];
#pragma unroll
                for (int w = 0; w < 3; ++w) {
                    const float4 ra = red[0][w][lane + 64 * i], rb = red[1][w][lane + 64 * i];
                    a.x += ra.x; a.y += ra.y; a.z += ra.z; a.w += ra.w;
                    b.x += rb.x; b.y += rb.y; b.z += rb.z; b.w += rb.w;
                }
                *reinterpret_cast<float4*>(dgamma_part + (int64_t)blockIdx.x * part_ld + col[i]) = a;
                *reinterpret_cast<float4*>(dbeta_part + (int64_t)blockIdx.x * part_ld + col[i]) = b;
            }
        }
    }
}

template <typename Th, int MV>
__global__ __launch_bounds__(LN_THREADS) void ln_res_fwd_kernel(const Th* __restrict__ h, const float* __restrict__ gamma, const float* __restrict__ beta,
                                                               const float* __restrict__ x, const float* __restrict__ ls, const float* __restrict__ sample_scale,
                                                               int rows_per_sample, float* __restrict__ out, Th* __restrict__ out_act,
                                                               float* __restrict__ mean, float* __restrict__ rstd, int64_t rows, int C, float eps) {
    const int lane = threadIdx.x & 63, wave = threadIdx.x >> 6;
    const int nv = C >> 2;
    int col[MV];
    bool ok[MV];
    float4 g[MV], bb[MV], lv[MV];
#pragma unroll
    for (int i = 0; i < MV; ++i) {
        const int c4 = lane + 64 * i;
        ok[i] = c4 < nv;
        col[i] = 4 * (ok[i] ? c4 : nv - 1);
        g[i] = *reinterpret_cast<const float4*>(gamma + col[i]);
        bb[i] = *reinterpret_cast<const float4*>(beta + col[i]);
        lv[i] = *reinterpret_cast<const float4*>(ls + col[i]);
    }
    for (int64_t row = (int64_t)blockIdx.x * 4 + wave; row < rows; row += (int64_t)gridDim.x * 4) {
        float4 v[MV], xv[MV];
#pragma unroll
        for (int i = 0; i < MV; ++i) {
            v[i] = load4(h + row * C + col[i]);
            xv[i] = *reinterpret_cast<const float4*>(x + row * C + col[i]);
        }
        const float sc = sample_scale ? sample_scale[(uint32_t)row / (uint32_t)rows_per_sample] : 1.0f;
        float s = 0.f;
// ... 209 lines not shown
        atomicAdd(out + n, s.x); atomicAdd(out + n + 1, s.y); atomicAdd(out + n + 2, s.z); atomicAdd(out + n + 3, s.w);
    }
}

int ln_grid(int64_t rows) {
    int64_t nb = (rows + 3) / 4;
    return (int)(nb < 2048 ? nb : 2048);
}

#define MTP_LN_MV(C_, CALL)                                      \
    do {                                                         \
        const int mv_ = (int)(((C_) / 4 + 63) / 64);             \
        if (mv_ <= 1) { CALL(1); }                               \
        else if (mv_ == 2) { CALL(2); }                          \
        else if (mv_ == 3) { CALL(3); }                          \
        else if (mv_ == 4) { CALL(4); }                          \
        else if (mv_ <= 6) { CALL(6); }                          \
        else { CALL(8); }                                        \
    } while (0)

template <typename Tx, typename Ty>
int launch_ln_fwd(const void* x, const float* g, const float* b, void* y, float* mean, float* rstd, int64_t rows, int64_t C, float eps, int gelu, hipStream_t s) {
    dim3 grid(ln_grid(rows)), block(LN_THREADS);
#define MTP_CALL(MV_)                                                                                                                                        \
    if (gelu)                                                                                                                                                \
        hipLaunchKernelGGL((ln_fwd_kernel<Tx, Ty, true, MV_>), grid, block, 0, s, (const Tx*)x, g, b, (Ty*)y, mean, rstd, rows, (int)C, eps);                \
    else                                                                                                                                                     \
        hipLaunchKernelGGL((ln_fwd_kernel<Tx, Ty, false, MV_>), grid, block, 0, s, (const Tx*)x, g, b, (Ty*)y, mean, rstd, rows, (int)C, eps)
    MTP_LN_MV(C, MTP_CALL);
#undef MTP_CALL
    return mtp_launch_status();
}

template <typename Tact, typename Tx, typename Tdx>
int launch_ln_bwd(const void* dy, const void* x, const float* mean, const float* rstd, const float* gamma, const float* beta, int gelu,
                  const float* dres, const float* extra, void* dx, void* dx_copy, const float* copy_scale, int64_t rps,
                  float* dgp, float* dbp, int64_t part_ld, int64_t rows, int64_t C, hipStream_t s, const float* win_add = nullptr, LnWin wg = LnWin{1, 1, 0, 0, 1, 1}) {
    dim3 grid((unsigned)mtp_layernorm_bwd_partial_rows(rows)), block(LN_THREADS);
#define MTP_CALL(MV_)                                                                                                                                        \
    if (gelu)                                                                                                                                                \
        hipLaunchKernelGGL((ln_bwd_kernel<Tact, Tx, Tdx, true, MV_>), grid, block, 0, s, (const Tact*)dy, (const Tx*)x, mean, rstd, gamma, beta, dres, extra, \
                           (Tdx*)dx, (Tact*)dx_copy, copy_scale, (int)(rps > 0 ? rps : 1), dgp, dbp, part_ld, rows, (int)C, win_add, wg);                    \
    else                                                                                                                                                     \
        hipLaunchKernelGGL((ln_bwd_kernel<Tact, Tx, Tdx, false, MV_>), grid, block, 0, s, (const Tact*)dy, (const Tx*)x, mean, rstd, gamma, beta, dres, extra, \
                           (Tdx*)dx, (Tact*)dx_copy, copy_scale, (int)(rps > 0 ? rps : 1), dgp, dbp, part_ld, rows, (int)C, win_add, wg)
    MTP_LN_MV(C, MTP_CALL);
#undef MTP_CALL
    return mtp_launch_status();
}

}

extern "C" int mtp_layernorm_fwd(const void* x, int x_dtype, const float* gamma, const float* beta, void* y, int y_dtype,
                                 float* mean, float* rstd, int64_t rows, int64_t C, float eps, int fuse_gelu, mtp_stream_t stream) {
    if (!x || !gamma || !beta || !y || rows <= 0 || C <= 0 || (C % 4) || C > 256 * MAXV) return MTP_ERR_ARG;
    hipStream_t s = (hipStream_t)stream;
    if (x_dtype == MTP_F32 && y_dtype == MTP_F32) return launch_ln_fwd<float, float>(x, gamma, beta, y, mean, rstd, rows, C, eps, fuse_gelu, s);
    if (x_dtype == MTP_F32 && y_dtype == MTP_BF16) return launch_ln_fwd<float, bf16_t>(x, gamma, beta, y, mean, rstd, rows, C, eps, fuse_gelu, s);
    if (x_dtype == MTP_BF16 && y_dtype == MTP_BF16) return launch_ln_fwd<bf16_t, bf16_t>(x, gamma, beta, y, mean, rstd, rows, C, eps, fuse_gelu, s);
    if (x_dtype == MTP_BF16 && y_dtype == MTP_F32) return launch_ln_fwd<bf16_t, float>(x, gamma, beta, y, mean, rstd, rows, C, eps, fuse_gelu, s);
    return MTP_ERR_UNSUPPORTED;
}

template <typename Th>
static int launch_ln_res(bool fwd, const void* a0, const void* h, const float* mean_c, float* mean, const float* rstd_c, float* rstd, const float* gamma, const float* beta,
                         const float* x, const float* ls, const float* ss, int rps, float* out, void* oact, void* dh, float* part, int64_t rows, int64_t C, float eps,
                         hipStream_t s) {
    if (fwd) {
        const dim3 grid(ln_grid(rows)), block(LN_THREADS);
#define MTP_CALL(MV_) hipLaunchKernelGGL((ln_res_fwd_kernel<Th, MV_>), grid, block, 0, s, (const Th*)h, gamma, beta, x, ls, ss, rps, out, (Th*)oact, mean, rstd, rows, (int)C, eps)
        MTP_LN_MV(C, MTP_CALL);
#undef MTP_CALL
    } else {
        const dim3 grid((unsigned)mtp_layernorm_bwd_partial_rows(rows)), block(LN_THREADS);
#define MTP_CALL(MV_) hipLaunchKernelGGL((ln_res_bwd_kernel<Th, MV_>), grid, block, 0, s, (const float*)a0, (const Th*)h, mean_c, rstd_c, gamma, beta, ls, ss, rps, (Th*)dh, part, rows, (int)C)
        MTP_LN_MV(C, MTP_CALL);
#undef MTP_CALL
    }
// ... 19 lines not shown
    const int rps = (int)(rows_per_sample > 0 ? rows_per_sample : 1);
    if (dtype == MTP_BF16) return launch_ln_res<bf16_t>(false, dout, h, mean, nullptr, rstd, nullptr, gamma, beta, nullptr, layer_scale, sample_scale, rps, nullptr, nullptr, dh, part, rows, C, 0.f, (hipStream_t)stream);
    if (dtype == MTP_F32) return launch_ln_res<float>(false, dout, h, mean, nullptr, rstd, nullptr, gamma, beta, nullptr, layer_scale, sample_scale, rps, nullptr, nullptr, dh, part, rows, C, 0.f, (hipStream_t)stream);
    return MTP_ERR_UNSUPPORTED;
}

extern "C" int64_t mtp_layernorm_bwd_partial_rows(int64_t rows) {
    const int64_t nb = (rows + 3) / 4;
    const int64_t cap = rows > 262144 ? 2048 : rows > 65536 ? 1024 : 512;
    return nb < cap ? nb : cap;
}

extern "C" int mtp_layernorm_bwd(const void* dy, int dy_dtype, const void* x, int x_dtype, const float* mean, const float* rstd,
                                 const float* gamma, const float* beta, int fuse_gelu, const float* dres, const float* extra, void* dx, int dx_dtype,
                                 void* dx_copy, int copy_dtype, const float* copy_scale, int64_t rows_per_sample,
                                 float* dgamma_part, float* dbeta_part, int64_t part_ld, int64_t rows, int64_t C, mtp_stream_t stream) {
    if (part_ld == 0) part_ld = C;
    if (part_ld < C || (part_ld % 4)) return MTP_ERR_ARG;
    if (!dy || !x || !mean || !rstd || !gamma || !dx || !dgamma_part || !dbeta_part || rows <= 0 || rows > INT32_MAX || (C % 4) || C > 256 * MAXV) return MTP_ERR_ARG;
    if (fuse_gelu && !beta) return MTP_ERR_ARG;
    if (dx_copy && copy_dtype != dy_dtype) return MTP_ERR_ARG;
    hipStream_t s = (hipStream_t)stream;
    if (dy_dtype == MTP_BF16 && x_dtype == MTP_F32 && dx_dtype == MTP_F32)
        return launch_ln_bwd<bf16_t, float, float>(dy, x, mean, rstd, gamma, beta, fuse_gelu, dres, extra, dx, dx_copy, copy_scale, rows_per_sample, dgamma_part, dbeta_part, part_ld, rows, C, s);
    if (dy_dtype == MTP_F32 && x_dtype == MTP_F32 && dx_dtype == MTP_F32)
        return launch_ln_bwd<float, float, float>(dy, x, mean, rstd, gamma, beta, fuse_gelu, dres, extra, dx, dx_copy, copy_scale, rows_per_sample, dgamma_part, dbeta_part, part_ld, rows, C, s);
    if (dy_dtype == MTP_BF16 && x_dtype == MTP_BF16 && dx_dtype == MTP_BF16)
        return launch_ln_bwd<bf16_t, bf16_t, bf16_t>(dy, x, mean, rstd, gamma, beta, fuse_gelu, dres, extra, dx, dx_copy, copy_scale, rows_per_sample, dgamma_part, dbeta_part, part_ld, rows, C, s);
    if (dy_dtype == MTP_F32 && x_dtype == MTP_BF16 && dx_dtype == MTP_BF16)
        return launch_ln_bwd<float, bf16_t, bf16_t>(dy, x, mean, rstd, gamma, beta, fuse_gelu, dres, extra, dx, dx_copy, copy_scale, rows_per_sample, dgamma_part, dbeta_part, part_ld, rows, C, s);
    return MTP_ERR_UNSUPPORTED;
}

extern "C" int mtp_layernorm_bwd_win(const void* dy, int dy_dtype, const void* x, int x_dtype, const float* mean, const float* rstd,
                                     const float* gamma, const float* dres, const float* extra, void* dx, int dx_dtype,
                                     void* dx_copy, int copy_dtype, const float* copy_scale, int64_t rows_per_sample,
                                     float* dgamma_part, float* dbeta_part, int64_t part_ld, int64_t rows, int64_t C,
                                     const float* win_add, int64_t B, int64_t Hp, int64_t Wp, mtp_stream_t stream) {
    if (part_ld == 0) part_ld = C;
    if (part_ld < C || (part_ld % 4)) return MTP_ERR_ARG;
    if (!dy || !x || !mean || !rstd || !gamma || !dx || !dgamma_part || !dbeta_part || rows <= 0 || rows > INT32_MAX || (C % 4) || C > 256 * MAXV) return MTP_ERR_ARG;
    if (!win_add || B <= 0 || Hp <= 0 || Wp <= 0 || B * Hp * Wp != rows) return MTP_ERR_ARG;
    if (dx_copy && copy_dtype != dy_dtype) return MTP_ERR_ARG;
    const int pad_h = (int)((7 - Hp % 7) % 7), pad_w = (int)((7 - Wp % 7) % 7);
    const LnWin wg = {(int)Hp, (int)Wp, pad_h / 2, pad_w / 2, (int)((Hp + pad_h) / 7), (int)((Wp + pad_w) / 7)};
    hipStream_t s = (hipStream_t)stream;
    if (dy_dtype == MTP_BF16 && x_dtype == MTP_F32 && dx_dtype == MTP_F32)
        return launch_ln_bwd<bf16_t, float, float>(dy, x, mean, rstd, gamma, nullptr, 0, dres, extra, dx, dx_copy, copy_scale, rows_per_sample, dgamma_part, dbeta_part, part_ld, rows, C, s, win_add, wg);
    if (dy_dtype == MTP_F32 && x_dtype == MTP_F32 && dx_dtype == MTP_F32)
        return launch_ln_bwd<float, float, float>(dy, x, mean, rstd, gamma, nullptr, 0, dres, extra, dx, dx_copy, copy_scale, rows_per_sample, dgamma_part, dbeta_part, part_ld, rows, C, s, win_add, wg);
    return MTP_ERR_UNSUPPORTED;
}

extern "C" int mtp_reduce_rows_f32(const float* part, int64_t ld, float* out, int64_t rows, int64_t C, int accumulate, mtp_stream_t stream) {
    if (!part || !out || rows <= 0 || C <= 0 || ld < C) return MTP_ERR_ARG;
    hipStream_t s = (hipStream_t)stream;
    if (!accumulate) {
        hipError_t e = hipMemsetAsync(out, 0, sizeof(float) * (size_t)C, s);
        if (e != hipSuccess) return (int)e;
    }
    const int64_t col_blocks = (C + 255) / 256;
    int64_t splits = 1024 / col_blocks;
    if (splits < 1) splits = 1;
    if (splits > rows) splits = rows;
    const int64_t rpb = (rows + splits - 1) / splits;
    splits = (rows + rpb - 1) / rpb;
// ... 100 lines not shown
```

### mtp_amd/engine.py

```python
import os

import torch

from . import ops
from .engine_base import EngineBase

F32 = torch.float32


class _Blk:
    __slots__ = ("window", "pre", "wqkv", "wqkvT", "wproj", "wprojT", "w1", "w1T", "w2", "w2T", "wsamp", "bsamp", "bproj", "b2", "wproj_s", "w2_s")


class BackboneEngine(EngineBase):
    def __init__(self, module, act_dtype=torch.bfloat16):
        super().__init__(module, act_dtype)
        self.C = module.embed_dim
        self.depth = len(module.blocks)
        self.heads = module.num_heads
        self.hd = self.C // self.heads
        self.scale = module.qk_scale if module.qk_scale is not None else self.hd ** -0.5
        self.window = [bool(w) for w in module.window_blocks]
        self.out_indices = list(module.out_indices)
        self._blk = None
# ... 45 lines not shown
            if ls:
                b.wproj_s, b.w2_s = torch.empty_like(P[pre + "attn.proj.weight"]), torch.empty_like(P[pre + "mlp.fc2.weight"])
                b.bproj, b.b2 = torch.empty_like(P[pre + "attn.proj.bias"]), torch.empty_like(P[pre + "mlp.fc2.bias"])
                self._ls.append((pre, b))
                b.wproj, b.wprojT = both(b.wproj_s)
            else:
                b.wproj, b.wprojT = both(P[pre + "attn.proj.weight"])
            b.w1, b.w1T = both(P[pre + "mlp.fc1.weight"])
            b.w2, b.w2T = both(b.w2_s if ls else P[pre + "mlp.fc2.weight"])
            if b.window:
                b.wsamp = torch.empty(5 * H, C, device=dev, dtype=F32)
                b.bsamp = torch.empty(5 * H, device=dev, dtype=F32)
                r0 = 0
                for head, rows in (("sampling_offsets", 2 * H), ("sampling_scales", 2 * H), ("sampling_angles", H)):
                    entries.append((P[pre + "attn.%s.2.weight" % head].detach().view(rows, C), b.wsamp[r0:r0 + rows], None, True))
                    entries.append((P[pre + "attn.%s.2.bias" % head].detach().view(1, rows), b.bsamp[r0:r0 + rows], None, True))
                    r0 += rows
            blks.append(b)
        self._blk = blks
        wpe = P["patch_embed.proj.weight"].detach()
        self._pe = both(wpe.view(wpe.shape[0], -1))
        fpn = {}
        for name in ("fpn1.0", "fpn1.3", "fpn2.0"):
            if name + ".weight" in P:
                Cin, Cout = P[name + ".weight"].shape[:2]
                fpn[name] = (torch.empty(4 * Cout, Cin, device=dev, dtype=act), torch.empty(Cin, 4 * Cout, device=dev, dtype=act))
        self._fpn = fpn
        self._wimg = ops.WeightImages(entries, act)

    wgrad_side_stream = True
    wgrad_max_jobs = 8
    wgrad_keep = 2

    @staticmethod
    def _colsum(dy, out):
        return ops.colsum(dy, out, accumulate=True)

    def _ln_bwd(self, *args, **kw):
        return ops.layernorm_bwd(*args, accumulate=True, defer=self._ln_parts, **kw)

    def _full_rel(self, pre, Hp, Wp):
        h = self.P.get(pre + "attn.full_attn_rel_pos_h")
        if h is not None:
            w = self.P[pre + "attn.full_attn_rel_pos_w"]
            if h.shape[0] < 2 * Hp - 1 or w.shape[0] < 2 * Wp - 1:
                raise ValueError("%sattn.full_attn_rel_pos_h/w have %d / %d rows, a %d x %d token grid needs %d / %d (resize them like "
                                 "init_weights does, or build the model for this input size)" % (pre, h.shape[0], w.shape[0], Hp, Wp, 2 * Hp - 1, 2 * Wp - 1))
            return h[:2 * Hp - 1], w[:2 * Wp - 1]
        key = (Hp, Wp)
        if self._zero_rel.get(key) is None:
            self._zero_rel[key] = (torch.zeros(2 * Hp - 1, self.hd, device=self.dev, dtype=F32),
                                   torch.zeros(2 * Wp - 1, self.hd, device=self.dev, dtype=F32))
        return self._zero_rel[key]

    def _drop_scales(self, B, training):
        rates = [float(self.m.drop_path_rates[i]) for i in range(self.depth)]
        live = [training and r > 0.0 and self.m.blocks[i].training for i, r in enumerate(rates)]
        if not any(live):
            return [(None, None)] * self.depth
        keep = torch.tensor([1.0 - r for r in rates], dtype=F32).to(self.dev, non_blocking=True).view(self.depth, 1, 1)
        s = torch.floor(keep + torch.rand(self.depth, 2, B, device=self.dev, dtype=F32)) / keep
        return [(s[i, 0], s[i, 1]) if live[i] else (None, None) for i in range(self.depth)]

    def _block_fwd(self, i, x, B, Hp, Wp, dps, save):
        P, b, C, T, N = self.P, self._blk[i], self.C, x.shape[0], Hp * Wp
        pre = b.pre
        s = {}
        mean1, rstd1 = self._e(T, dtype=F32), self._e(T, dtype=F32)
        ln1 = ops.layernorm_fwd(x, P[pre + "norm1.weight"], P[pre + "norm1.bias"], self._e(T, C), mean1, rstd1)
        if b.window:
# ... 20 lines not shown
        h = ops.gemm_nt(ln2, b.w1, self._e(T, 4 * C), epi=ops.EPI_BIAS_GELU_DG, bias=P[pre + "mlp.fc1.bias"], aux=u)
        x2 = ops.gemm_nt(h, b.w2, self._e(T, C, dtype=F32), epi=ops.EPI_BIAS_RES, bias=b.b2, res=x1,
                         rowscale=dps[1], rows_per_sample=N)
        if save:
            s.update(x=x, mean1=mean1, rstd1=rstd1, ln1=ln1, qkv=qkv, o=o, lse=lse, x1=x1, mean2=mean2, rstd2=rstd2, ln2=ln2, u=u, h=h)
        return x2, s

    def _layer_scale_grads(self, pre, lin, gname, G):
        P = self.P
        gw, gb, gam = G[pre + lin + ".weight"], G[pre + lin + ".bias"], P[pre + gname]
        G[pre + gname].add_((gw * P[pre + lin + ".weight"]).sum(1) + gb * P[pre + lin + ".bias"])
        gw.mul_(gam[:, None])
        gb.mul_(gam)

    def _block_bwd(self, i, s, dx2, dx2_act, B, Hp, Wp, dps, G, extra, prev_scale):
        P, b, C, N = self.P, self._blk[i], self.C, Hp * Wp
        pre = b.pre
        T = dx2.shape[0]
        wq = self._wq
        ls = pre + "gamma_1" in G
        wq.add(dx2_act, s["h"], G[pre + "mlp.fc2.weight"], G[pre + "mlp.fc2.bias"], after=(lambda: self._layer_scale_grads(pre, "mlp.fc2", "gamma_2", G)) if ls else None,
               norm_ok=not ls)
        du = ops.gemm_nt(dx2_act, b.w2T, self._e(T, 4 * C), epi=ops.EPI_MUL, aux=s["u"])
        wq.add(du, s["ln2"], G[pre + "mlp.fc1.weight"], G[pre + "mlp.fc1.bias"])
        dln2 = ops.gemm_nt(du, b.w1T, self._e(T, C))
        del du
        dx1, dx1_act = self._e(T, C, dtype=F32), self._e(T, C)
        self._ln_bwd(dln2, s["x1"], s["mean2"], s["rstd2"], P[pre + "norm2.weight"], dx1, G[pre + "norm2.weight"], G[pre + "norm2.bias"],
                          dres=dx2, dx_copy=dx1_act, copy_scale=dps[0], rows_per_sample=N)
        wq.add(dx1_act, s["o"], G[pre + "attn.proj.weight"], G[pre + "attn.proj.bias"], after=(lambda: self._layer_scale_grads(pre, "attn.proj", "gamma_1", G)) if ls else None,
               norm_ok=not ls)
        do = ops.gemm_nt(dx1_act, b.wprojT, self._e(T, C))
        dqkv = self._e(T, 3 * C)
        if b.window:
            nh, nw = ops.rvsa_windows(Hp, Wp)
            R = B * nh * nw
            H = self.heads
            dsamp = self._e(R, 5 * H, dtype=F32)
            ops.rvsa_attn_bwd(s["qkv"], s["samp"], s["o"], do, s["lse"], dqkv, dsamp,
                              P[pre + "attn.rel_pos_h"], P[pre + "attn.rel_pos_w"], P[pre + "attn.relative_position_bias_table"],
                              G[pre + "attn.rel_pos_h"], G[pre + "attn.rel_pos_w"], G[pre + "attn.relative_position_bias_table"],
                              B, Hp, Wp, H, self.scale, accumulate=True, defer=self._ln_parts)
            names = ("sampling_offsets", "sampling_scales", "sampling_angles")
            self._sl_jobs.append((s["pooled"], dsamp, [G[pre + "attn.%s.2.weight" % n].view(-1, C) for n in names],
                                  [G[pre + "attn.%s.2.bias" % n] for n in names]))
        else:
            rel_h, rel_w = self._full_rel(pre, Hp, Wp)
            if pre + "attn.full_attn_rel_pos_h" in G:
                drel_h, drel_w = G[pre + "attn.full_attn_rel_pos_h"][:2 * Hp - 1], G[pre + "attn.full_attn_rel_pos_w"][:2 * Wp - 1]
            else:
                drel_h, drel_w = self._e(*rel_h.shape, dtype=F32), self._e(*rel_w.shape, dtype=F32)
            ops.full_attn_bwd(s["qkv"], s["o"], do, s["lse"], dqkv, rel_h, rel_w, drel_h, drel_w, B, Hp, Wp, self.heads, self.scale,
                              accumulate=True, defer=self._ln_parts)
        wq.add(dqkv, s["ln1"], G[pre + "attn.qkv.weight"], G[pre + "attn.qkv.bias"])
        win_add = None
        if b.window:
            win_add = ops.rvsa_sampling_bwd_win(dsamp, b.wsamp, s["avg"], self._e(*s["avg"].shape, dtype=F32))
        dln1 = ops.gemm_nt(dqkv, b.wqkvT, self._e(T, C))
        dx0, dx0_act = self._e(T, C, dtype=F32), self._e(T, C)
        self._ln_bwd(dln1, s["x"], s["mean1"], s["rstd1"], P[pre + "norm1.weight"], dx0, G[pre + "norm1.weight"], G[pre + "norm1.bias"],
                          dres=dx1, extra=extra, dx_copy=dx0_act, copy_scale=prev_scale, rows_per_sample=N,
                          **(dict(win_add=win_add, grid=(B, Hp, Wp)) if win_add is not None else {}))
        return dx0, dx0_act

    def forward(self, img, training=False, need_grad=False, feature_dtype=None):
        m = self.m
        self.dev = img.device
        self.prepare_weights()
        self.P = P = {k: v.detach() for k, v in self.params().items()}
        C, act = self.C, self.act
        ps = m.patch_size
        fdt = feature_dtype or act
        if img.dtype == torch.uint8:
            pp = getattr(m, "data_preprocessor", None)
            if pp is None:
                raise ValueError("uint8 input needs ViT_Win_RVSA_V3_WSZ7.set_data_preprocessor(mean, std, ...)")
            B, H, W, Cin = img.shape
            Hp, Wp = ops.padded_grid(H, W, ps, pp["pad_size_divisor"])
            N, T = Hp * Wp, B * Hp * Wp
            cols = ops.preprocess_patchify(img.contiguous(), self._e(T, Cin * ps * ps), ps, pp["mean"], pp["std"], pp["bgr_to_rgb"],
                                           pp["pad_size_divisor"], pp["pad_value"])
            H, W = Hp * ps, Wp * ps
        else:
            B, Cin, H, W = img.shape
            Hp, Wp = H // ps, W // ps
            N, T = Hp * Wp, B * Hp * Wp
            img = img.contiguous()
            if img.dtype != F32:
                img = img.float()
            cols = ops.patchify(img, self._e(T, Cin * ps * ps), ps)
# ... 57 lines not shown
            raise NotImplementedError("the reference defines the FPN tail for patch_size 16 and 8 only (VIT:640-670)")
        t0 = taps[0] if self.act == F32 else ops.cast(taps[0], self._e(T, C))
        y1 = ops.gemm_nt(t0, self._fpn["fpn1.0"][0], self._e(T, 4 * C), bias=P["fpn1.0.bias"], bias_mod=C)
        mean, rstd = self._e(4 * T, dtype=F32), self._e(4 * T, dtype=F32)
        g1 = ops.layernorm_fwd(y1.view(4 * T, C), P["fpn1.1.ln.weight"], P["fpn1.1.ln.bias"], self._e(4 * T, C), mean, rstd, gelu=True)
        y2 = ops.gemm_nt(g1, self._fpn["fpn1.3"][0], self._e(4 * T, 4 * C), bias=P["fpn1.3.bias"], bias_mod=C)
        feats.append(ops.tokens_to_nchw(y2.view(16 * T, C), self._e(B, C, 4 * Hp, 4 * Wp, dtype=fdt), B, Hp, Wp, 2))
        t1 = taps[1] if self.act == F32 else ops.cast(taps[1], self._e(T, C))
        z = ops.gemm_nt(t1, self._fpn["fpn2.0"][0], self._e(T, 4 * C), bias=P["fpn2.0.bias"], bias_mod=C)
        feats.append(ops.tokens_to_nchw(z.view(4 * T, C), self._e(B, C, 2 * Hp, 2 * Wp, dtype=fdt), B, Hp, Wp, 1))
        feats.append(ops.tokens_to_nchw(taps[2], self._e(B, C, Hp, Wp, dtype=fdt), B, Hp, Wp, 0))
        Ho, Wo = Hp // 2, Wp // 2
        pooled = ops.maxpool2_tokens_fwd(taps[3], self._e(B * Ho * Wo, C), B, Hp, Wp)
        feats.append(ops.tokens_to_nchw(pooled, self._e(B, C, Ho, Wo, dtype=fdt), B, Ho, Wo, 0))
        if need_grad:
            fctx = dict(t0=t0, y1=y1, mean=mean, rstd=rstd, g1=g1, t1=t1, tap3=taps[3])
        return feats, fctx

    def _convt_wgrad(self, dy, x, gw):
        dwg = self._e(dy.shape[1], x.shape[1], dtype=F32)
        self._wq.add(dy, x, dwg, after=lambda: ops.convt_unpack_grad(dwg, gw), norm_of=gw)

    def _fpn_bwd(self, dfeats, fctx, B, Hp, Wp, G):
        P, C, T, act = self.P, self.C, B * Hp * Wp, self.act
        out = [None] * 4

        def as_in(df):
            df = df.contiguous()
            return df if df.dtype in (F32, torch.bfloat16) else df.float()

        if fctx.get("p8"):
            H2, W2, H4, W4 = Hp // 2, Wp // 2, Hp // 4, Wp // 4
            if dfeats[0] is not None:
                dz = ops.nchw_to_tokens(as_in(dfeats[0]), self._e(4 * T, C), B, Hp, Wp, 1)
                self._convt_wgrad(dz.view(T, 4 * C), fctx["t0"], G["fpn1.0.weight"])
                self._colsum(dz, G["fpn1.0.bias"])
                out[0] = ops.gemm_nt(dz.view(T, 4 * C), self._fpn["fpn1.0"][1], self._e(T, C, dtype=F32))
            if dfeats[1] is not None:
                out[1] = ops.nchw_to_tokens(as_in(dfeats[1]), self._e(T, C, dtype=F32), B, Hp, Wp, 0)
            if dfeats[2] is not None:
                dp = ops.nchw_to_tokens(as_in(dfeats[2]), self._e(B * H2 * W2, C, dtype=F32), B, H2, W2, 0)
                out[2] = ops.maxpool2_tokens_bwd(fctx["tap2"], dp, self._e(T, C, dtype=F32), B, Hp, Wp)
            if dfeats[3] is not None:
                dq2 = ops.nchw_to_tokens(as_in(dfeats[3]), self._e(B * H4 * W4, C, dtype=F32), B, H4, W4, 0)
                dq1 = ops.maxpool2_tokens_bwd(fctx["q1"], dq2, self._e(B * H2 * W2, C, dtype=F32), B, H2, W2)
                out[3] = ops.maxpool2_tokens_bwd(fctx["tap3"], dq1, self._e(T, C, dtype=F32), B, Hp, Wp)
            return out

        if dfeats[0] is not None:
            dy2 = ops.nchw_to_tokens(as_in(dfeats[0]), self._e(16 * T, C), B, Hp, Wp, 2)
            self._convt_wgrad(dy2.view(4 * T, 4 * C), fctx["g1"], G["fpn1.3.weight"])
            self._colsum(dy2, G["fpn1.3.bias"])
            dg1 = ops.gemm_nt(dy2.view(4 * T, 4 * C), self._fpn["fpn1.3"][1], self._e(4 * T, C))
            dy1 = self._e(4 * T, C)
            self._ln_bwd(dg1, fctx["y1"].view(4 * T, C), fctx["mean"], fctx["rstd"], P["fpn1.1.ln.weight"], dy1,
                              G["fpn1.1.ln.weight"], G["fpn1.1.ln.bias"], beta=P["fpn1.1.ln.bias"], gelu=True)
            self._convt_wgrad(dy1.view(T, 4 * C), fctx["t0"], G["fpn1.0.weight"])
            self._colsum(dy1, G["fpn1.0.bias"])
            out[0] = ops.gemm_nt(dy1.view(T, 4 * C), self._fpn["fpn1.0"][1], self._e(T, C, dtype=F32))
        if dfeats[1] is not None:
            dz = ops.nchw_to_tokens(as_in(dfeats[1]), self._e(4 * T, C), B, Hp, Wp, 1)
            self._convt_wgrad(dz.view(T, 4 * C), fctx["t1"], G["fpn2.0.weight"])
            self._colsum(dz, G["fpn2.0.bias"])
            out[1] = ops.gemm_nt(dz.view(T, 4 * C), self._fpn["fpn2.0"][1], self._e(T, C, dtype=F32))
        if dfeats[2] is not None:
            out[2] = ops.nchw_to_tokens(as_in(dfeats[2]), self._e(T, C, dtype=F32), B, Hp, Wp, 0)
        if dfeats[3] is not None:
            Ho, Wo = Hp // 2, Wp // 2
            dp = ops.nchw_to_tokens(as_in(dfeats[3]), self._e(B * Ho * Wo, C, dtype=F32), B, Ho, Wo, 0)
            out[3] = ops.maxpool2_tokens_bwd(fctx["tap3"], dp, self._e(T, C, dtype=F32), B, Hp, Wp)
        return out

    def backward(self, ctx, dfeats, G, need_input_grad=False, on_block_done=None, split_last=False, sqn=None):
        B, Cin, H, W, Hp, Wp = ctx["geom"]
        C, N, T = self.C, Hp * Wp, B * Hp * Wp
        P = self.P
        self.dev = ctx["cols"].device
        wq = self._begin_backward(sqn)
        if ctx["fctx"].get("taps_only"):
            dtaps = [None if d is None else ops.nchw_to_tokens((d.contiguous() if d.dtype in (F32, torch.bfloat16) else d.float().contiguous()),
                                                               self._e(T, C, dtype=F32), B, Hp, Wp, 0) for d in dfeats]
        else:
            dtaps = self._fpn_bwd(dfeats, ctx["fctx"], B, Hp, Wp, G)
        tapgrad = {}
        last, dps, saved = ctx["last"], ctx["dps"], ctx["saved"]
        if ctx.get("final") is not None:
            dsum = None
            for d in dtaps:
                if d is None:
                    continue
                if dsum is None:
                    dsum = d
                else:
                    ops.axpy(dsum, d)
            if dsum is not None:
                xl, fm, fr = ctx["final"]
# ... 43 lines not shown
```

### mtp_amd/ops.py

```python
import ctypes as C

import torch

from . import _lib
from ._lib import (EPI_BIAS, EPI_BIAS_GELU, EPI_BIAS_GELU_DG, EPI_BIAS_RES, EPI_DGELU, EPI_MUL, MTP_BF16, MTP_F32, GemmArgs,
                   check)
from ._lib import (GEMM_NT_FAMILY_P8, GEMM_NT_FAMILY_REG, GEMM_NT_FAMILY_SB, GEMM_NT_FAMILY_SB8, GEMM_NT_FAMILY_STRIP, GEMM_NT_NO_P8,
                   GEMM_NT_NO_PERSIST, GEMM_NT_NO_SB8, GEMM_NT_NO_STRIP, GEMM_NT_P8, GEMM_NT_P8_224, GEMM_NT_P8_256, GEMM_NT_PERSIST,
                   GEMM_NT_REG_STAGED, GEMM_NT_SB8, GEMM_NT_STRIP, GEMM_ORDER_GROUPED, GEMM_ORDER_PLAIN, GEMM_ORDER_ROW_MAJOR, GEMM_STORE_NT,
                   GEMM_STORE_PLAIN, GEMM_STORE_SC1, GEMM_TN_REG_TRANSPOSE, GEMM_TN_TR_FULL_ONLY, GEMM_TNG_PLAIN_ORDER, GEMM_TNG_PLAIN_PHASES)

_DT = {torch.float32: MTP_F32, torch.bfloat16: MTP_BF16}
def lib():
    return _lib.load()


def _dt(t):
    try:
        return _DT[t.dtype]
    except KeyError:
        raise TypeError("mtp_amd ops take float32 / bfloat16 tensors, got %s" % t.dtype)


def _p(t):
# ... 238 lines not shown
                g.in_dtype, g.out_dtype, g.variant = MTP_BF16, MTP_F32, self.variant
                if splits > 1:
                    g.split_k, g.aux = splits, _p(part)
                if use_sqn:
                    g.workspace, g.workspace_bytes = _p(self.sqn), 4
                if cs is not None:
                    assert cs.dtype == torch.float32 and cs.numel() == M and cs.is_contiguous()
                    g.colsum = _p(cs)
            check(lib().mtp_gemm_tn_grouped(arr, len(chunk), _s()), "mtp_gemm_tn_grouped")
        after, self.after = self.after, []
        for fn in after:
            fn()
        self.tiles = 0


def sum_partials(jobs):
    while jobs:
        chunk, jobs[:] = jobs[:12], jobs[12:]
        n = len(chunk)
        P = C.c_void_p * n
        parts, outs = P(*[j[0].data_ptr() for j in chunk]), P(*[j[1].data_ptr() for j in chunk])
        numel, splits = (C.c_int64 * n)(*[j[2] for j in chunk]), (C.c_int * n)(*[j[3] for j in chunk])
        check(lib().mtp_sum_partials_batch(parts, outs, numel, splits, n, _s()), "mtp_sum_partials_batch")


def layernorm_fwd(x, gamma, beta, y, mean=None, rstd=None, eps=1e-6, gelu=False):
    rows, Cc = x.shape
    check(lib().mtp_layernorm_fwd(_p(x), _dt(x), _f32(gamma), _f32(beta), _p(y), _dt(y), _f32(mean), _f32(rstd),
                                  rows, Cc, eps, int(gelu), _s()), "mtp_layernorm_fwd")
    return y


def layernorm_bwd(dy, x, mean, rstd, gamma, dx, dgamma, dbeta, beta=None, gelu=False, dres=None, extra=None,
                  dx_copy=None, copy_scale=None, rows_per_sample=0, accumulate=False, defer=None, win_add=None, grid=None):
    rows, Cc = x.shape
    nblk = lib().mtp_layernorm_bwd_partial_rows(rows)
    part = _scratch((nblk, 2 * Cc), x.device, torch.float32)
    if win_add is not None:
        B, Hp, Wp = grid
        nh, nw = rvsa_windows(Hp, Wp)
        assert not gelu and tuple(win_add.shape) == (B * nh * nw, Cc) and B * Hp * Wp == rows
        check(lib().mtp_layernorm_bwd_win(_p(dy), _dt(dy), _p(x), _dt(x), _f32(mean), _f32(rstd), _f32(gamma), _f32(dres), _f32(extra), _p(dx), _dt(dx),
                                          _p(dx_copy), (_dt(dx_copy) if dx_copy is not None else 0), _f32(copy_scale), rows_per_sample,
                                          part.data_ptr(), part.data_ptr() + 4 * Cc, 2 * Cc, rows, Cc, _f32(win_add), B, Hp, Wp, _s()), "mtp_layernorm_bwd_win")
    else:
        check(lib().mtp_layernorm_bwd(_p(dy), _dt(dy), _p(x), _dt(x), _f32(mean), _f32(rstd), _f32(gamma), _f32(beta), int(gelu),
                                      _f32(dres), _f32(extra), _p(dx), _dt(dx), _p(dx_copy), (_dt(dx_copy) if dx_copy is not None else 0),
                                      _f32(copy_scale), rows_per_sample, part.data_ptr(), part.data_ptr() + 4 * Cc, 2 * Cc, rows, Cc, _s()),
              "mtp_layernorm_bwd")
    if defer is not None and _adjacent(dgamma, dbeta) and dgamma.numel() == Cc:
        defer.append((part, dgamma, accumulate))
    else:
        _reduce_pair(part, Cc, dgamma, dbeta, accumulate)
    return dx


def layernorm_residual_fwd(h, gamma, beta, x, layer_scale, out, out_act, mean, rstd, sample_scale=None, rows_per_sample=0, eps=1e-6):
    rows, Cc = h.shape
    check(lib().mtp_layernorm_residual_fwd(_p(h), _dt(h), _f32(gamma), _f32(beta), _f32(x), _f32(layer_scale), _f32(sample_scale), rows_per_sample,
                                           _f32(out), _p(out_act), _f32(mean), _f32(rstd), rows, Cc, eps, _s()), "mtp_layernorm_residual_fwd")
    return out


def layernorm_residual_bwd(dout, h, mean, rstd, gamma, beta, layer_scale, dh, dgamma, dbeta, dls, sample_scale=None, rows_per_sample=0, defer=None):
    rows, Cc = h.shape
    nblk = lib().mtp_layernorm_bwd_partial_rows(rows)
    part = _scratch((nblk, 3 * Cc), h.device, torch.float32)
    check(lib().mtp_layernorm_residual_bwd(_f32(dout), _p(h), _dt(h), _f32(mean), _f32(rstd), _f32(gamma), _f32(beta), _f32(layer_scale), _f32(sample_scale),
                                           rows_per_sample, _p(dh), part.data_ptr(), rows, Cc, _s()), "mtp_layernorm_residual_bwd")
    pair = _adjacent(dgamma, dbeta) and dgamma.numel() == Cc
# ... 189 lines not shown
        self.table = torch.frombuffer(bytearray(bytes(arr)), dtype=torch.uint8).to(flat.data.device)
        self.lr = None if lr_of is None else torch.tensor(scales, dtype=torch.float32).to(flat.data.device)
        self.flat = flat
        return self

    def step(self, m, v, hyper, sqn, max_norm, grad_scale):
        f = self.flat
        if self.lr is not None:
            check(lib().mtp_adamw_weight_images_lr(self.table.data_ptr(), _f32(self.lr), self.n, self.total_tiles, self.act, _f32(f.data), _f32(f.grad), _f32(m), _f32(v),
                                                   _f32(hyper), _f32(sqn), max_norm, grad_scale, _s()), "mtp_adamw_weight_images_lr")
            return
        check(lib().mtp_adamw_weight_images(self.table.data_ptr(), self.n, self.total_tiles, self.act, _f32(f.data), _f32(f.grad), _f32(m), _f32(v), _f32(hyper),
                                            _f32(sqn), max_norm, grad_scale, _s()), "mtp_adamw_weight_images")


def convt_pack(w, wg, wgT):
    Cin, Cout = w.shape[:2]
    dt = _dt(wg if wg is not None else wgT)
    check(lib().mtp_convt_pack(_f32(w), _p(wg), _p(wgT), dt, Cin, Cout, _s()), "mtp_convt_pack")


def convt_unpack_grad(dwg, dw):
    Cin, Cout = dw.shape[:2]
    check(lib().mtp_convt_unpack_grad(_f32(dwg), _f32(dw), Cin, Cout, _s()), "mtp_convt_unpack_grad")
    return dw


def tokens_to_nchw(x, out, B, Hp, Wp, levels):
    Cc = x.shape[-1]
    check(lib().mtp_tokens_to_nchw(_p(x), _dt(x), _p(out), _dt(out), B, Hp, Wp, Cc, levels, _s()), "mtp_tokens_to_nchw")
    return out


def nchw_to_tokens(f, out, B, Hp, Wp, levels):
    Cc = f.shape[1]
    check(lib().mtp_nchw_to_tokens(_p(f), _dt(f), _p(out), _dt(out), B, Hp, Wp, Cc, levels, _s()), "mtp_nchw_to_tokens")
    return out


def maxpool2_tokens_fwd(x, y, B, Hp, Wp):
    check(lib().mtp_maxpool2_tokens_fwd(_f32(x), _p(y), _dt(y), B, Hp, Wp, x.shape[-1], _s()), "mtp_maxpool2_tokens_fwd")
    return y


def maxpool2_tokens_bwd(x, dy, dx, B, Hp, Wp, accumulate=False):
    check(lib().mtp_maxpool2_tokens_bwd(_f32(x), _p(dy), _dt(dy), _f32(dx), int(accumulate), B, Hp, Wp, x.shape[-1], _s()), "mtp_maxpool2_tokens_bwd")
    return dx


def axpy(y, x, alpha=1.0):
    check(lib().mtp_axpy_f32(_f32(y), _f32(x), alpha, y.numel(), _s()), "mtp_axpy_f32")
    return y


def scale_rows_cast(src, dst, scale=None, rows_per_sample=0):
    rows, Cc = src.shape
    check(lib().mtp_scale_rows_cast(_f32(src), _p(dst), _dt(dst), _f32(scale), rows_per_sample, rows, Cc, _s()), "mtp_scale_rows_cast")
    return dst


def full_attn_fwd(qkv, o, lse, rel_h, rel_w, B, Hp, Wp, heads, scale):
    hd = qkv.shape[1] // (3 * heads)
    check(lib().mtp_full_attn_fwd(_p(qkv), _p(o), _f32(lse), _dt(qkv), _f32(rel_h), _f32(rel_w), B, Hp, Wp, heads, hd, scale, _s()), "mtp_full_attn_fwd")
    return o, lse


def full_attn_bwd(qkv, o, dout, lse, dqkv, rel_h, rel_w, drel_h, drel_w, B, Hp, Wp, heads, scale, accumulate=False, defer=None):
    hd = qkv.shape[1] // (3 * heads)
# ... 79 lines not shown
    rows = (C.c_int64 * n)(*[d.shape[0] for d in dws])
    P = C.c_void_p * n
    check(lib().mtp_small_linear_dw_segments(_f32(x), _f32(dy), R, dy.shape[1], K, n, rows, P(*[_f32(d) for d in dws]), P(*[_f32(d) for d in dbs]), _s()),
          "mtp_small_linear_dw_segments")


SL_BATCH = 8


def small_linear_dw_segments_flush(jobs):
    groups = {}
    for x, dy, dws, dbs in jobs:
        groups.setdefault((tuple(x.shape), tuple(dy.shape), tuple(d.shape[0] for d in dws)), []).append((x, dy, dws, dbs))
    for ((R, K), (_, N), rows_), g in groups.items():
        nseg = len(rows_)
        rows = (C.c_int64 * nseg)(*rows_)
        for i0 in range(0, len(g), SL_BATCH):
            chunk = g[i0:i0 + SL_BATCH]
            n = len(chunk)
            P, PS = C.c_void_p * n, C.c_void_p * (n * nseg)
            check(lib().mtp_small_linear_dw_segments_batched(P(*[_f32(c[0]) for c in chunk]), P(*[_f32(c[1]) for c in chunk]), n, R, N, K, nseg, rows,
                                                             PS(*[_f32(d) for c in chunk for d in c[2]]), PS(*[_f32(d) for c in chunk for d in c[3]]), _s()),
                  "mtp_small_linear_dw_segments_batched")
    del jobs[:]


def rvsa_attn_fwd(qkv, samp, o, lse, rel_h, rel_w, table, B, Hp, Wp, heads, scale):
    hd = qkv.shape[1] // (3 * heads)
    check(lib().mtp_rvsa_attn_fwd(_p(qkv), _f32(samp), _p(o), _f32(lse), _dt(qkv), _f32(rel_h), _f32(rel_w), _f32(table),
                                  B, Hp, Wp, heads, hd, scale, _s()), "mtp_rvsa_attn_fwd")
    return o, lse


def rvsa_attn_bwd(qkv, samp, o, dout, lse, dqkv, dsamp, rel_h, rel_w, table, drel_h, drel_w, dtable, B, Hp, Wp, heads, scale, accumulate=False, defer=None):
    hd = qkv.shape[1] // (3 * heads)
    T, C3 = qkv.shape
    Cc = C3 // 3
    nh, nw = rvsa_windows(Hp, Wp)
    nblk = B * nh * nw * heads
    dev = qkv.device
    dkv = _scratch((T, 2 * Cc), dev, torch.float32)
    rel_part = _scratch((nblk, 26 * hd), dev, torch.float32)
    tab_part = _scratch((B * nh * nw, heads * 169), dev, torch.float32)
    check(lib().mtp_rvsa_attn_bwd(_p(qkv), _f32(samp), _p(o), _p(dout), _f32(lse), _p(dqkv), _p(dkv), _f32(dsamp), _p(rel_part), _p(tab_part),
                                  _dt(qkv), _f32(rel_h), _f32(rel_w), _f32(table), B, Hp, Wp, heads, hd, scale, _s()), "mtp_rvsa_attn_bwd")
    if defer is not None and _adjacent(drel_h, drel_w) and drel_h.numel() == 13 * hd:
        defer.append((rel_part, drel_h, accumulate))
        defer.append((tab_part, dtable, accumulate, (heads, 169)))
        return dqkv
    _reduce_pair(rel_part, 13 * hd, drel_h, drel_w, accumulate)
    check(lib().mtp_reduce_rows_t_f32(_p(tab_part), tab_part.shape[1], _f32(dtable), tab_part.shape[0], heads, 169, int(accumulate), _s()),
          "mtp_reduce_rows_t_f32")
    return dqkv


def zero_segments(base, start, count):
    assert base.dtype == torch.float32 and start.dtype == torch.int64 and count.dtype == torch.int64 and start.numel() == count.numel()
    check(lib().mtp_zero_segments_f32(_p(base), start.data_ptr(), count.data_ptr(), start.numel(), _s()), "mtp_zero_segments_f32")


def sqnorm(g, out):
    check(lib().mtp_sqnorm_f32(_f32(g), _f32(out), g.numel(), _s()), "mtp_sqnorm_f32")
    return out


def sqnorm_segments(base, start, count, out):
    assert base.dtype == torch.float32 and start.dtype == torch.int64 and count.dtype == torch.int64 and start.numel() == count.numel()
    check(lib().mtp_sqnorm_segments_f32(_p(base), start.data_ptr(), count.data_ptr(), start.numel(), _f32(out), _s()), "mtp_sqnorm_segments_f32")
    return out


def adamw_flat(p, g, m, v, seg_start, seg_wd, hyper, sqn=None, max_norm=0.0, grad_scale=1.0):
    assert seg_start.dtype == torch.int64 and seg_start.is_cuda
    check(lib().mtp_adamw_flat(_f32(p), _f32(g), _f32(m), _f32(v), p.numel(), seg_start.data_ptr(), _f32(seg_wd), seg_start.numel(),
                               _f32(hyper), _f32(sqn), max_norm, grad_scale, _s()), "mtp_adamw_flat")


def adamw_flat_lr(p, g, m, v, seg_start, seg_wd, seg_lr, hyper, sqn=None, max_norm=0.0, grad_scale=1.0):
# ... 536 lines not shown
```

Measured before the change: 1883 images/sec.

## Fuse RVSA window sampling backward into scatter kernel and bias colsums into producers

```diff
diff --git a/include/mtp_hip.h b/include/mtp_hip.h
--- a/include/mtp_hip.h
+++ b/include/mtp_hip.h
@@ -110,6 +110,11 @@
                       const float* dres, const float* extra, void* dx, int dx_dtype,
                       void* dx_copy, int copy_dtype, const float* copy_scale, int64_t rows_per_sample,
                       float* dgamma_part, float* dbeta_part, int64_t part_ld, int64_t rows, int64_t C, mtp_stream_t stream);
+int mtp_layernorm_bwd_dxsum(const void* dy, int dy_dtype, const void* x, int x_dtype, const float* mean, const float* rstd,
+                            const float* gamma, const float* beta, int fuse_gelu,
+                            const float* dres, const float* extra, void* dx, int dx_dtype,
+                            void* dx_copy, int copy_dtype, const float* copy_scale, int64_t rows_per_sample,
+                            float* dgamma_part, float* dbeta_part, float* dxsum_part, int64_t part_ld, int64_t rows, int64_t C, mtp_stream_t stream);
 int mtp_layernorm_bwd_win(const void* dy, int dy_dtype, const void* x, int x_dtype, const float* mean, const float* rstd,
                           const float* gamma, const float* dres, const float* extra, void* dx, int dx_dtype,
                           void* dx_copy, int copy_dtype, const float* copy_scale, int64_t rows_per_sample,
@@ -155,6 +160,8 @@
 int mtp_convt_unpack_grad(const float* dwg, float* dw, int64_t Cin, int64_t Cout, mtp_stream_t stream);
 int mtp_tokens_to_nchw(const void* x, int x_dtype, void* out, int out_dtype, int64_t B, int64_t Hp, int64_t Wp, int64_t C, int levels, mtp_stream_t stream);
 int mtp_nchw_to_tokens(const void* f, int f_dtype, void* out, int out_dtype, int64_t B, int64_t Hp, int64_t Wp, int64_t C, int levels, mtp_stream_t stream);
+int mtp_nchw_to_tokens_colsum(const void* f, int f_dtype, void* out, int out_dtype, int64_t B, int64_t Hp, int64_t Wp, int64_t C, int levels, float* colsum,
+                              mtp_stream_t stream);
 int mtp_maxpool2_tokens_fwd(const float* x, void* y, int y_dtype, int64_t B, int64_t Hp, int64_t Wp, int64_t C, mtp_stream_t stream);
 int mtp_maxpool2_tokens_bwd(const float* x, const void* dy, int dy_dtype, float* dx, int accumulate, int64_t B, int64_t Hp, int64_t Wp, int64_t C, mtp_stream_t stream);
 int mtp_axpy_f32(float* y, const float* x, float alpha, int64_t n, mtp_stream_t stream);
@@ -245,6 +252,11 @@
                       void* dqkv, float* dkv_f32, float* dsamp, float* rel_part, float* tab_part, int dtype,
                       const float* rel_h, const float* rel_w, const float* bias_table,
                       int64_t B, int64_t Hp, int64_t Wp, int64_t heads, int64_t hd, float scale, mtp_stream_t stream);
+int mtp_rvsa_attn_bwd_win(const void* qkv, const float* samp, const void* o, const void* dout, const float* lse,
+                          void* dqkv, float* dkv_f32, float* dsamp, float* rel_part, float* tab_part, int dtype,
+                          const float* rel_h, const float* rel_w, const float* bias_table,
+                          int64_t B, int64_t Hp, int64_t Wp, int64_t heads, int64_t hd, float scale,
+                          const float* wsamp, const float* avg, float* g, mtp_stream_t stream);
 
 int mtp_zero_segments_f32(float* base, const int64_t* start, const int64_t* count, int n, mtp_stream_t stream);
 int mtp_sqnorm_f32(const float* g, float* out, int64_t n, mtp_stream_t stream);
diff --git a/mtp_amd/_lib.py b/mtp_amd/_lib.py
--- a/mtp_amd/_lib.py
+++ b/mtp_amd/_lib.py
@@ -79,6 +79,7 @@
     "mtp_layernorm_fwd": (i32, [p, i32, p, p, p, i32, p, p, i64, i64, f32, i32, p]),
     "mtp_layernorm_bwd_partial_rows": (i64, [i64]),
     "mtp_layernorm_bwd": (i32, [p, i32, p, i32, p, p, p, p, i32, p, p, p, i32, p, i32, p, i64, p, p, i64, i64, i64, p]),
+    "mtp_layernorm_bwd_dxsum": (i32, [p, i32, p, i32, p, p, p, p, i32, p, p, p, i32, p, i32, p, i64, p, p, p, i64, i64, i64, p]),
     "mtp_reduce_rows_f32": (i32, [p, i64, p, i64, i64, i32, p]),
     "mtp_reduce_rows_batched_f32": (i32, [p, p, i32, i64, i64, i64, i32, p]),
     "mtp_reduce_rows_t_f32": (i32, [p, i64, p, i64, i64, i64, i32, p]),
@@ -95,6 +96,7 @@
     "mtp_convt_unpack_grad": (i32, [p, p, i64, i64, p]),
     "mtp_tokens_to_nchw": (i32, [p, i32, p, i32, i64, i64, i64, i64, i32, p]),
     "mtp_nchw_to_tokens": (i32, [p, i32, p, i32, i64, i64, i64, i64, i32, p]),
+    "mtp_nchw_to_tokens_colsum": (i32, [p, i32, p, i32, i64, i64, i64, i64, i32, p, p]),
     "mtp_maxpool2_tokens_fwd": (i32, [p, p, i32, i64, i64, i64, i64, p]),
     "mtp_maxpool2_tokens_bwd": (i32, [p, p, i32, p, i32, i64, i64, i64, i64, p]),
     "mtp_axpy_f32": (i32, [p, p, f32, i64, p]),
@@ -142,6 +144,7 @@
     "mtp_small_linear_dw_segments_batched": (i32, [p, p, i32, i64, i64, i64, i32, p, p, p, p]),
     "mtp_rvsa_attn_fwd": (i32, [p, p, p, p, i32, p, p, p, i64, i64, i64, i64, i64, f32, p]),
     "mtp_rvsa_attn_bwd": (i32, [p, p, p, p, p, p, p, p, p, p, i32, p, p, p, i64, i64, i64, i64, i64, f32, p]),
+    "mtp_rvsa_attn_bwd_win": (i32, [p, p, p, p, p, p, p, p, p, p, i32, p, p, p, i64, i64, i64, i64, i64, f32, p, p, p, p]),
     "mtp_zero_segments_f32": (i32, [p, p, p, i32, p]),
     "mtp_sqnorm_f32": (i32, [p, p, i64, p]),
     "mtp_sqnorm_segments_f32": (i32, [p, p, p, i32, p, p]),
diff --git a/mtp_amd/csrc/attn.hip b/mtp_amd/csrc/attn.hip
--- a/mtp_amd/csrc/attn.hip
+++ b/mtp_amd/csrc/attn.hip
@@ -855,10 +855,11 @@
     return mtp_launch_status();
 }
 
-extern "C" int mtp_rvsa_attn_bwd(const void* qkv, const float* samp, const void* o, const void* dout, const float* lse,
-                                 void* dqkv, float* dkv_f32, float* dsamp, float* rel_part, float* tab_part, int dtype,
-                                 const float* rel_h, const float* rel_w, const float* bias_table,
-                                 int64_t B, int64_t Hp, int64_t Wp, int64_t heads, int64_t hd, float scale, mtp_stream_t stream) {
+static int rvsa_attn_bwd_impl(const void* qkv, const float* samp, const void* o, const void* dout, const float* lse,
+                              void* dqkv, float* dkv_f32, float* dsamp, float* rel_part, float* tab_part, int dtype,
+                              const float* rel_h, const float* rel_w, const float* bias_table,
+                              int64_t B, int64_t Hp, int64_t Wp, int64_t heads, int64_t hd, float scale,
+                              const float* wsamp, const float* avg, float* gwin, mtp_stream_t stream) {
     if (!qkv || !samp || !o || !dout || !lse || !dqkv || !dkv_f32 || !dsamp || !rel_part || !tab_part || !rel_h || !rel_w || !bias_table) return MTP_ERR_ARG;
     if (B <= 0 || Hp < 7 || Wp < 7 || heads <= 0) return MTP_ERR_ARG;
     if (hd != HD) return MTP_ERR_UNSUPPORTED;
@@ -866,8 +867,16 @@
     const int64_t Ttok = B * Hp * Wp, C = heads * HD;
     hipStream_t s = (hipStream_t)stream;
     const int family = rvsa_bwd_family(dtype, Hp, Wp, heads);
-    if (family == MTP_RVSA_BWD_MFMA_DENSE)
-        return mtp_rvsa_bwd_mfma_launch(qkv, samp, o, dout, lse, dqkv, dkv_f32, dsamp, rel_part, tab_part, rel_h, rel_w, bias_table, B, Hp, Wp, heads, scale, s);
+    const int64_t windows = B * g.nh * g.nw, nsamp = 5 * heads;
+    if (family == MTP_RVSA_BWD_MFMA_DENSE) {
+        const int64_t cblks = (C / 4 + 64 * RVSA_WIN_Q - 1) / (64 * RVSA_WIN_Q);
+        if (gwin && nsamp <= 4096 && windows * cblks <= INT32_MAX / 2) {
+            const RvsaWinAddend wa = {wsamp, avg, gwin, (int)C, (int)nsamp, (int)(windows * cblks), 0};
+            return mtp_rvsa_bwd_mfma_launch(qkv, samp, o, dout, lse, dqkv, dkv_f32, dsamp, rel_part, tab_part, rel_h, rel_w, bias_table, B, Hp, Wp, heads, scale, s, &wa);
+        }
+        const int rc = mtp_rvsa_bwd_mfma_launch(qkv, samp, o, dout, lse, dqkv, dkv_f32, dsamp, rel_part, tab_part, rel_h, rel_w, bias_table, B, Hp, Wp, heads, scale, s);
+        return (rc || !gwin) ? rc : mtp_rvsa_sampling_bwd_win(dsamp, wsamp, avg, gwin, windows, C, nsamp, stream);
+    }
     hipError_t e = hipMemsetAsync(dkv_f32, 0, sizeof(float) * (size_t)(Ttok * 2 * C), s);
     if (e != hipSuccess) return (int)e;
     dim3 grid((unsigned)(B * g.nh * g.nw * heads)), block(64);
@@ -882,5 +891,24 @@
                            dkv_f32, dsamp, rel_part, tab_part, rel_h, rel_w, bias_table, g, scale);
         hipLaunchKernelGGL((dkv_convert_kernel<float>), cgrid, cblock, 0, s, dkv_f32, (float*)dqkv, Ttok, (int)C);
     }
-    return mtp_launch_status();
-}
+    const int rc = mtp_launch_status();
+    return (rc || !gwin) ? rc : mtp_rvsa_sampling_bwd_win(dsamp, wsamp, avg, gwin, windows, C, nsamp, stream);
+}
+
+extern "C" int mtp_rvsa_attn_bwd(const void* qkv, const float* samp, const void* o, const void* dout, const float* lse,
+                                 void* dqkv, float* dkv_f32, float* dsamp, float* rel_part, float* tab_part, int dtype,
+                                 const float* rel_h, const float* rel_w, const float* bias_table,
+                                 int64_t B, int64_t Hp, int64_t Wp, int64_t heads, int64_t hd, float scale, mtp_stream_t stream) {
+    return rvsa_attn_bwd_impl(qkv, samp, o, dout, lse, dqkv, dkv_f32, dsamp, rel_part, tab_part, dtype, rel_h, rel_w, bias_table, B, Hp, Wp, heads, hd, scale,
+                              nullptr, nullptr, nullptr, stream);
+}
+
+extern "C" int mtp_rvsa_attn_bwd_win(const void* qkv, const float* samp, const void* o, const void* dout, const float* lse,
+                                     void* dqkv, float* dkv_f32, float* dsamp, float* rel_part, float* tab_part, int dtype,
+                                     const float* rel_h, const float* rel_w, const float* bias_table,
+                                     int64_t B, int64_t Hp, int64_t Wp, int64_t heads, int64_t hd, float scale,
+                                     const float* wsamp, const float* avg, float* g, mtp_stream_t stream) {
+    if (!wsamp || !avg || !g) return MTP_ERR_ARG;
+    return rvsa_attn_bwd_impl(qkv, samp, o, dout, lse, dqkv, dkv_f32, dsamp, rel_part, tab_part, dtype, rel_h, rel_w, bias_table, B, Hp, Wp, heads, hd, scale,
+                              wsamp, avg, g, stream);
+}
diff --git a/mtp_amd/csrc/attn_launch.h b/mtp_amd/csrc/attn_launch.h
--- a/mtp_amd/csrc/attn_launch.h
+++ b/mtp_amd/csrc/attn_launch.h
@@ -4,9 +4,16 @@
 
 int mtp_rvsa_fwd_mfma_launch(const void* qkv, const float* samp, void* o, float* lse, const float* rel_h, const float* rel_w, const float* bias_table,
                              int64_t B, int64_t Hp, int64_t Wp, int64_t heads, float scale, hipStream_t s);
+struct RvsaWinAddend {
+    const float* w;
+    const float* avg;
+    float* g;
+    int C, N, count, first_x;
+};
+constexpr int RVSA_WIN_Q = 4;
 int mtp_rvsa_bwd_mfma_launch(const void* qkv, const float* samp, const void* o, const void* dout, const float* lse, void* dqkv, float* dkv, float* dsamp,
                              float* rel_part, float* tab_part, const float* rel_h, const float* rel_w, const float* bias_table,
-                             int64_t B, int64_t Hp, int64_t Wp, int64_t heads, float scale, hipStream_t s);
+                             int64_t B, int64_t Hp, int64_t Wp, int64_t heads, float scale, hipStream_t s, const RvsaWinAddend* win = nullptr);
 int mtp_rvsa_bwd_mfma_scatter_mode(int64_t Hp, int64_t Wp, int64_t heads);
 bool mtp_full_v3_fits(int64_t Hp, int64_t Wp);
 int mtp_full_fwd_flash_keys(int64_t Hp, int64_t Wp);
diff --git a/mtp_amd/csrc/attn_rvsa_bwd4.hip b/mtp_amd/csrc/attn_rvsa_bwd4.hip
--- a/mtp_amd/csrc/attn_rvsa_bwd4.hip
+++ b/mtp_amd/csrc/attn_rvsa_bwd4.hip
@@ -840,14 +840,23 @@
 constexpr int SCB = 224;
 
 __global__ __launch_bounds__(256, 2) void rvsa_scatter_gemm_kernel(const bf16_t* __restrict__ dsel, const float* __restrict__ samp, bf16_t* __restrict__ dqkv,
-                                                                  RvsaGeom g) {
+                                                                  RvsaGeom g, const float* __restrict__ dsamp, RvsaWinAddend wa) {
     __shared__ __attribute__((aligned(16))) char Kimg[SCB * 128];
     __shared__ __attribute__((aligned(16))) char Vimg[SCB * 128];
     __shared__ __attribute__((aligned(16))) float xs[SCB];
     __shared__ __attribute__((aligned(16))) float ys[SCB];
+    if ((int)blockIdx.x < wa.first_x) {
+        static_assert(sizeof(float4) * 4 * 64 * RVSA_WIN_Q <= SCB * 128 && sizeof(float) * 4096 <= SCB * 128, "the addend's LDS lives in the K / V images");
+        const int id = (int)blockIdx.x * (int)gridDim.y + (int)blockIdx.y;
+        if (id >= wa.count) return;
+        const int cblks = (wa.C / 4 + 64 * RVSA_WIN_Q - 1) / (64 * RVSA_WIN_Q);
+        rvsa_win_addend<RVSA_WIN_Q>(dsamp, wa.w, wa.avg, wa.g, wa.C, wa.N, id / cblks, id % cblks, reinterpret_cast<float*>(Vimg), reinterpret_cast<float4*>(Kimg));
+        return;
+    }
     const int tid = threadIdx.x, lane = tid & 63, wave = tid >> 6, fr = lane & 15, gq = lane >> 4;
     const int H = g.heads, nW = g.nh * g.nw, S = nW * 49;
-    const int h = blockIdx.x % H, b = blockIdx.x / H;
+    const int bx = (int)blockIdx.x - wa.first_x;
+    const int h = bx % H, b = bx / H;
     const int C = H * HD, N = g.Hp * g.Wp;
     const int t0 = blockIdx.y * SCB, nt = (N - t0) < SCB ? (N - t0) : SCB;
     const int64_t ld = 3 * (int64_t)C;
@@ -971,9 +980,10 @@
 
 int mtp_rvsa_bwd_mfma_launch(const void* qkv, const float* samp, const void* o, const void* dout, const float* lse, void* dqkv, float* dkv, float* dsamp,
                              float* rel_part, float* tab_part, const float* rel_h, const float* rel_w, const float* bias_table,
-                             int64_t B, int64_t Hp, int64_t Wp, int64_t heads, float scale, hipStream_t s) {
+                             int64_t B, int64_t Hp, int64_t Wp, int64_t heads, float scale, hipStream_t s, const RvsaWinAddend* win) {
     const RvsaGeom g = make_geom(Hp, Wp, heads);
     const int mode = mtp_rvsa_bwd_mfma_scatter_mode(Hp, Wp, heads);
+    if (win && (mode != 4 || win->N > 4096 || win->count <= 0)) return MTP_ERR_ARG;
     const dim3 grid((unsigned)(B * g.nh * g.nw * heads));
     if (mode == 4) {
         static const bool old4 = []() { const char* e = getenv("MTP_RVSA_BWD"); return e && e[0] == '4'; }();
@@ -984,7 +994,12 @@
             hipLaunchKernelGGL(rvsa_bwd5_mfma_kernel, grid, dim3(256), 0, s, (const bf16_t*)qkv, samp, (const bf16_t*)o, (const bf16_t*)dout, lse,
                                (bf16_t*)dqkv, dkv, dsamp, rel_part, tab_part, rel_h, rel_w, bias_table, g, scale);
         const int64_t N = Hp * Wp;
-        hipLaunchKernelGGL(rvsa_scatter_gemm_kernel, dim3((unsigned)(B * heads), (unsigned)((N + SCB - 1) / SCB)), dim3(256), 0, s, (const bf16_t*)dkv, samp, (bf16_t*)dqkv, g);
+        const unsigned bands = (unsigned)((N + SCB - 1) / SCB);
+        RvsaWinAddend wa = win ? *win : RvsaWinAddend{nullptr, nullptr, nullptr, 0, 0, 0, 0};
+        const unsigned extra_x = win ? ((unsigned)wa.count + bands - 1) / bands : 0u;
+        wa.first_x = (int)extra_x;
+        hipLaunchKernelGGL(rvsa_scatter_gemm_kernel, dim3((unsigned)(B * heads) + extra_x, bands), dim3(256), 0, s, (const bf16_t*)dkv, samp, (bf16_t*)dqkv, g,
+                           (const float*)dsamp, wa);
     } else {
         hipLaunchKernelGGL(rvsa_bwd4_mfma_kernel<1>, grid, dim3(256), 0, s, (const bf16_t*)qkv, samp, (const bf16_t*)o, (const bf16_t*)dout, lse,
                            (bf16_t*)dqkv, dkv, dsamp, rel_part, tab_part, rel_h, rel_w, bias_table, g, scale);
diff --git a/mtp_amd/csrc/common.h b/mtp_amd/csrc/common.h
--- a/mtp_amd/csrc/common.h
+++ b/mtp_amd/csrc/common.h
@@ -158,6 +158,48 @@
     return v;
 }
 
+template <int Q>
+__device__ __forceinline__ void rvsa_win_addend(const float* __restrict__ dsamp, const float* __restrict__ w, const float* __restrict__ avg, float* __restrict__ g,
+                                                int C, int N, int win, int cblk, float* __restrict__ ds, float4* __restrict__ part) {
+    const int lane = threadIdx.x & 63, q = threadIdx.x >> 6;
+    int c4[Q];
+    bool live[Q];
+    float4 d[Q];
+#pragma unroll
+    for (int j = 0; j < Q; ++j) {
+        c4[j] = (cblk * Q + j) * 64 + lane;
+        live[j] = c4[j] < C / 4;
+        if (!live[j]) c4[j] = 0;
+        d[j] = make_float4(0, 0, 0, 0);
+    }
+    for (int n = threadIdx.x; n < N; n += 256) ds[n] = dsamp[(int64_t)win * N + n];
+    __syncthreads();
+    const int nq = (N + 3) / 4, n0 = q * nq, n1 = (n0 + nq) < N ? (n0 + nq) : N;
+#pragma unroll 10
+    for (int n = n0; n < n1; ++n) {
+        const float t = ds[n];
+#pragma unroll
+        for (int j = 0; j < Q; ++j) {
+            const float4 ww = load4(w + (int64_t)n * C + 4 * c4[j]);
+            d[j].x += t * ww.x; d[j].y += t * ww.y; d[j].z += t * ww.z; d[j].w += t * ww.w;
+        }
+    }
+#pragma unroll
+    for (int j = 0; j < Q; ++j) part[(q * Q + j) * 64 + lane] = d[j];
+    __syncthreads();
+    if (q) return;
+    const float k = 1.0f / 49.0f;
+#pragma unroll
+    for (int j = 0; j < Q; ++j) {
+        if (!live[j]) continue;
+        const float4 p0 = part[j * 64 + lane], p1 = part[(Q + j) * 64 + lane], p2 = part[(2 * Q + j) * 64 + lane], p3 = part[(3 * Q + j) * 64 + lane];
+        const float4 s = make_float4((p0.x + p1.x) + (p2.x + p3.x), (p0.y + p1.y) + (p2.y + p3.y), (p0.z + p1.z) + (p2.z + p3.z), (p0.w + p1.w) + (p2.w + p3.w));
+        const float4 a = load4(avg + (int64_t)win * C + 4 * c4[j]);
+        *reinterpret_cast<float4*>(g + (int64_t)win * C + 4 * c4[j]) =
+            make_float4(s.x * (a.x > 0 ? k : 0.01f * k), s.y * (a.y > 0 ? k : 0.01f * k), s.z * (a.z > 0 ? k : 0.01f * k), s.w * (a.w > 0 ? k : 0.01f * k));
+    }
+}
+
 static inline int mtp_optin_lds(const void* kern, int bytes, unsigned long long& mask) {
     int dev = 0;
     if (hipGetDevice(&dev) != hipSuccess) dev = 64;
diff --git a/mtp_amd/csrc/elementwise.hip b/mtp_amd/csrc/elementwise.hip
--- a/mtp_amd/csrc/elementwise.hip
+++ b/mtp_amd/csrc/elementwise.hip
@@ -43,9 +43,74 @@
     return r;
 }
 
-template <typename Tin, typename Tout, bool ROWS2COLS>
-__global__ __launch_bounds__(256) void transpose_kernel(const Tin* __restrict__ in, Tout* __restrict__ out, int64_t S, int64_t C, int Wp, int L) {
+constexpr int TR_WALK = 16;
+template <bool ON> struct TrColsum {};
+template <> struct TrColsum<true> {
+    float* sum;
+    int ntile;
+    int64_t total;
+    int nct;
+    int walks;
+};
+
+__device__ __forceinline__ int pixel_to_row32(int s, int Wp, int L) {
+    if (L == 0) return s;
+    const uint32_t Wo = (uint32_t)Wp << L;
+    const int y = (int)((uint32_t)s / Wo), x = (int)((uint32_t)s - (uint32_t)y * Wo);
+    int r = (y >> L) * Wp + (x >> L);
+    for (int l = 1; l <= L; ++l) r = r * 4 + (((y >> (L - l)) & 1) << 1) + ((x >> (L - l)) & 1);
+    return r;
+}
+
+template <typename Tin, typename Tout, bool ROWS2COLS, bool COLSUM = false>
+__global__ __launch_bounds__(256) void transpose_kernel(const Tin* __restrict__ in, Tout* __restrict__ out, int64_t S, int64_t C, int Wp, int L, TrColsum<COLSUM> cs) {
     __shared__ float tile[64][65];
+    if constexpr (COLSUM) {
+        static_assert(!ROWS2COLS, "the column sums belong to the NCHW -> tokens direction");
+        const int64_t c0 = (int64_t)(blockIdx.x % (uint32_t)cs.nct) * 64;
+        const int t = threadIdx.x, a = t >> 2, g = (t & 3) * 16;
+        const int64_t c = c0 + a;
+        const int64_t f0 = (int64_t)(blockIdx.x / (uint32_t)cs.nct);
+        float acc = 0.f;
+        for (int64_t f = f0; f < cs.total; f += cs.walks) {
+            const int64_t bt = f / cs.ntile, ti = f - bt * cs.ntile, s0 = ti * 64;
+            const Tin* ib = in + bt * S * C;
+            Tout* ob = out + bt * S * C;
+            if (c < C) {
+                const Tin* rp = ib + c * S + s0 + g;
+#pragma unroll
+                for (int v = 0; v < 4; ++v) {
+                    const int64_t s2 = s0 + g + 4 * v;
+                    if (s2 + 3 < S && (S & 3) == 0) {
+                        const float4 x = load4(rp + 4 * v);
+                        tile[a][g + 4 * v] = x.x; tile[a][g + 4 * v + 1] = x.y; tile[a][g + 4 * v + 2] = x.z; tile[a][g + 4 * v + 3] = x.w;
+                        acc += x.x; acc += x.y; acc += x.z; acc += x.w;
+                    } else {
+                        for (int e = 0; e < 4; ++e)
+                            if (s2 + e < S) {
+                                const float x = Elem<Tin>::load(rp + 4 * v + e);
+                                tile[a][g + 4 * v + e] = x;
+                                acc += x;
+                            }
+                    }
+                }
+            }
+            __syncthreads();
+            const int64_t s = s0 + a;
+            if (s < S) {
+                Tout* wp = ob + pixel_to_row(s, Wp, L) * C + c0 + g;
+#pragma unroll
+                for (int v = 0; v < 4; ++v)
+                    if (c0 + g + 4 * v < C)
+                        store4(wp + 4 * v, make_float4(tile[g + 4 * v][a], tile[g + 4 * v + 1][a], tile[g + 4 * v + 2][a], tile[g + 4 * v + 3][a]));
+            }
+            __syncthreads();
+        }
+        acc += lane_xor<1>(acc);
+        acc += lane_xor<2>(acc);
+        if ((t & 3) == 0 && c < C) atomicAdd(cs.sum + c, acc);
+        return;
+    }
     const int64_t bt = blockIdx.z;
     const int64_t s0 = (int64_t)blockIdx.x * 64, c0 = (int64_t)blockIdx.y * 64;
     const Tin* ib = in + bt * S * C;
@@ -107,9 +172,72 @@
     }
 }
 
-template <bool ROWS2COLS>
-__global__ __launch_bounds__(256) void transpose8_bf16_kernel(const bf16_t* __restrict__ in, bf16_t* __restrict__ out, int64_t S, int64_t C, int Wp, int L) {
+template <bool ROWS2COLS, bool COLSUM = false>
+__global__ __launch_bounds__(256) void transpose8_bf16_kernel(const bf16_t* __restrict__ in, bf16_t* __restrict__ out, int64_t S, int64_t C, int Wp, int L, TrColsum<COLSUM> cs) {
     __shared__ float tile[64][65];
+    if constexpr (COLSUM) {
+        static_assert(!ROWS2COLS, "the column sums belong to the NCHW -> tokens direction");
+        const int c0 = (int)(blockIdx.x % (uint32_t)cs.nct) * 64, Ci = (int)C, Si = (int)S;
+        const int t = threadIdx.x, ra = t >> 3, cg = (t & 7) * 8;
+        const uint32_t f0 = blockIdx.x / (uint32_t)cs.nct, total = (uint32_t)cs.total, walks = (uint32_t)cs.walks;
+        const int nwalk = (int)((total - f0 + walks - 1) / walks);
+        int bt = (int)(f0 / (uint32_t)cs.ntile), ti = (int)(f0 - (uint32_t)bt * (uint32_t)cs.ntile);
+        const int dbt = (int)(walks / (uint32_t)cs.ntile), dti = (int)(walks - (uint32_t)dbt * (uint32_t)cs.ntile);
+        const bool cok[2] = {c0 + ra < Ci, c0 + ra + 32 < Ci};
+        const int crow[2] = {cok[0] ? c0 + ra : Ci - 1, cok[1] ? c0 + ra + 32 : Ci - 1};
+        float acc[2] = {0.f, 0.f};
+        uint4 raw[2];
+        bool rok[2];
+        auto fetch = [&](int b, int tile) {
+            const bool sok = tile * 64 + cg < Si;
+            const int so = sok ? tile * 64 + cg : 0;
+#pragma unroll
+            for (int h = 0; h < 2; ++h) {
+                raw[h] = *reinterpret_cast<const uint4*>(in + ((int64_t)b * C + crow[h]) * S + so);
+                rok[h] = sok && cok[h];
+            }
+        };
+        fetch(bt, ti);
+        for (int k = 0; k < nwalk; ++k) {
+#pragma unroll
+            for (int h = 0; h < 2; ++h) {
+                const uint4 v = rok[h] ? raw[h] : make_uint4(0u, 0u, 0u, 0u);
+                const float x[8] = {bf16_bits_to_f32(v.x & 0xffffu), bf16_bits_to_f32(v.x >> 16), bf16_bits_to_f32(v.y & 0xffffu), bf16_bits_to_f32(v.y >> 16),
+                                    bf16_bits_to_f32(v.z & 0xffffu), bf16_bits_to_f32(v.z >> 16), bf16_bits_to_f32(v.w & 0xffffu), bf16_bits_to_f32(v.w >> 16)};
+#pragma unroll
+                for (int e = 0; e < 8; ++e) {
+                    tile[ra + 32 * h][cg + e] = x[e];
+                    acc[h] += x[e];
+                }
+            }
+            __syncthreads();
+            const int b = bt, s0 = ti * 64;
+            bt += dbt; ti += dti;
+            if (ti >= cs.ntile) { ti -= cs.ntile; ++bt; }
+            if (k + 1 < nwalk) fetch(bt, ti);
+            bf16_t* ob = out + (int64_t)b * S * C;
+#pragma unroll
+            for (int h = 0; h < 2; ++h) {
+                const int sp = s0 + ra + 32 * h;
+                if (sp < Si && c0 + cg < Ci) {
+                    float y[8];
+#pragma unroll
+                    for (int e = 0; e < 8; ++e) y[e] = tile[cg + e][ra + 32 * h];
+                    store8(ob + (int64_t)pixel_to_row32(sp, Wp, L) * C + c0 + cg, y);
+                }
+            }
+            __syncthreads();
+        }
+#pragma unroll
+        for (int h = 0; h < 2; ++h) {
+            float v = acc[h];
+            v += lane_xor<1>(v);
+            v += lane_xor<2>(v);
+            v += lane_xor<4>(v);
+            if ((t & 7) == 0 && cok[h]) atomicAdd(cs.sum + c0 + ra + 32 * h, v);
+        }
+        return;
+    }
     const int64_t bt = blockIdx.z;
     const int64_t s0 = (int64_t)blockIdx.x * 64, c0 = (int64_t)blockIdx.y * 64;
     const bf16_t* ib = in + bt * S * C;
@@ -164,10 +292,31 @@
     if (C % 4) return MTP_ERR_ARG;
     dim3 grid((unsigned)((S + 63) / 64), (unsigned)((C + 63) / 64), (unsigned)batches), block(256);
     if (in_dt == MTP_BF16 && out_dt == MTP_BF16 && !(S & 7) && !(C & 7) && !(((uintptr_t)in | (uintptr_t)out) & 15)) {
-        hipLaunchKernelGGL((transpose8_bf16_kernel<ROWS2COLS>), grid, block, 0, s, (const bf16_t*)in, (bf16_t*)out, S, C, Wp, L);
+        hipLaunchKernelGGL((transpose8_bf16_kernel<ROWS2COLS>), grid, block, 0, s, (const bf16_t*)in, (bf16_t*)out, S, C, Wp, L, TrColsum<false>{});
         return mtp_launch_status();
     }
-#define MTP_TR(TI, TO) hipLaunchKernelGGL((transpose_kernel<TI, TO, ROWS2COLS>), grid, block, 0, s, (const TI*)in, (TO*)out, S, C, Wp, L)
+#define MTP_TR(TI, TO) hipLaunchKernelGGL((transpose_kernel<TI, TO, ROWS2COLS>), grid, block, 0, s, (const TI*)in, (TO*)out, S, C, Wp, L, TrColsum<false>{})
+    if (in_dt == MTP_F32 && out_dt == MTP_F32) MTP_TR(float, float);
+    else if (in_dt == MTP_F32 && out_dt == MTP_BF16) MTP_TR(float, bf16_t);
+    else if (in_dt == MTP_BF16 && out_dt == MTP_F32) MTP_TR(bf16_t, float);
+    else if (in_dt == MTP_BF16 && out_dt == MTP_BF16) MTP_TR(bf16_t, bf16_t);
+    else return MTP_ERR_UNSUPPORTED;
+#undef MTP_TR
+    return mtp_launch_status();
+}
+
+int launch_nchw_to_tokens_colsum(const void* in, int in_dt, void* out, int out_dt, int64_t batches, int64_t S, int64_t C, int Wp, int L, float* colsum, hipStream_t s) {
+    if (C % 4) return MTP_ERR_ARG;
+    const int64_t ntile = (S + 63) / 64, total = batches * ntile;
+    const int64_t nct = (C + 63) / 64, walks = (total + TR_WALK - 1) / TR_WALK;
+    if (S > INT32_MAX || C > INT32_MAX || total > INT32_MAX || walks * nct > INT32_MAX) return MTP_ERR_ARG;
+    const TrColsum<true> cs = {colsum, (int)ntile, total, (int)nct, (int)walks};
+    dim3 grid((unsigned)(walks * nct)), block(256);
+    if (in_dt == MTP_BF16 && out_dt == MTP_BF16 && !(S & 7) && !(C & 7) && !(((uintptr_t)in | (uintptr_t)out) & 15)) {
+        hipLaunchKernelGGL((transpose8_bf16_kernel<false, true>), grid, block, 0, s, (const bf16_t*)in, (bf16_t*)out, S, C, Wp, L, cs);
+        return mtp_launch_status();
+    }
+#define MTP_TR(TI, TO) hipLaunchKernelGGL((transpose_kernel<TI, TO, false, true>), grid, block, 0, s, (const TI*)in, (TO*)out, S, C, Wp, L, cs)
     if (in_dt == MTP_F32 && out_dt == MTP_F32) MTP_TR(float, float);
     else if (in_dt == MTP_F32 && out_dt == MTP_BF16) MTP_TR(float, bf16_t);
     else if (in_dt == MTP_BF16 && out_dt == MTP_F32) MTP_TR(bf16_t, float);
@@ -983,6 +1132,12 @@
     return launch_transpose<false>(f, f_dtype, out, out_dtype, B, (Hp * Wp) << (2 * levels), C, (int)Wp, levels, (hipStream_t)stream);
 }
 
+extern "C" int mtp_nchw_to_tokens_colsum(const void* f, int f_dtype, void* out, int out_dtype, int64_t B, int64_t Hp, int64_t Wp, int64_t C, int levels, float* colsum,
+                                         mtp_stream_t stream) {
+    if (!f || !out || !colsum || B <= 0 || Hp <= 0 || Wp <= 0 || levels < 0 || levels > 4) return MTP_ERR_ARG;
+    return launch_nchw_to_tokens_colsum(f, f_dtype, out, out_dtype, B, (Hp * Wp) << (2 * levels), C, (int)Wp, levels, colsum, (hipStream_t)stream);
+}
+
 extern "C" int mtp_maxpool2_tokens_fwd(const float* x, void* y, int y_dtype, int64_t B, int64_t Hp, int64_t Wp, int64_t C, mtp_stream_t stream) {
     if (!x || !y || B <= 0 || Hp < 2 || Wp < 2 || (C % 4)) return MTP_ERR_ARG;
     dim3 grid(blocks_for(B * (Hp / 2) * (Wp / 2) * C / 4, 256, 8192)), block(256);
@@ -1158,32 +1313,8 @@
 __global__ __launch_bounds__(256) void rvsa_sampling_bwd_win_kernel(const float* __restrict__ dsamp, const float* __restrict__ w, const float* __restrict__ avg,
                                                                    float* __restrict__ g, int C, int N) {
     extern __shared__ __attribute__((aligned(16))) float ds[];
-    __shared__ float4 part[4][64];
-    const int win = blockIdx.x;
-    const int lane = threadIdx.x & 63, q = threadIdx.x >> 6;
-    const int c4 = blockIdx.y * 64 + lane;
-    const bool live = c4 < C / 4;
-    for (int n = threadIdx.x; n < N; n += 256) ds[n] = dsamp[(int64_t)win * N + n];
-    __syncthreads();
-    const int nq = (N + 3) / 4, n0 = q * nq, n1 = (n0 + nq) < N ? (n0 + nq) : N;
-    float4 d = make_float4(0, 0, 0, 0);
-    if (live) {
-#pragma unroll 10
-        for (int n = n0; n < n1; ++n) {
-            const float4 ww = load4(w + (int64_t)n * C + 4 * c4);
-            const float t = ds[n];
-            d.x += t * ww.x; d.y += t * ww.y; d.z += t * ww.z; d.w += t * ww.w;
-        }
-    }
-    part[q][lane] = d;
-    __syncthreads();
-    if (!live || q) return;
-    const float4 p0 = part[0][lane], p1 = part[1][lane], p2 = part[2][lane], p3 = part[3][lane];
-    d = make_float4((p0.x + p1.x) + (p2.x + p3.x), (p0.y + p1.y) + (p2.y + p3.y), (p0.z + p1.z) + (p2.z + p3.z), (p0.w + p1.w) + (p2.w + p3.w));
-    const float4 a = load4(avg + (int64_t)win * C + 4 * c4);
-    const float k = 1.0f / 49.0f;
-    *reinterpret_cast<float4*>(g + (int64_t)win * C + 4 * c4) =
-        make_float4(d.x * (a.x > 0 ? k : 0.01f * k), d.y * (a.y > 0 ? k : 0.01f * k), d.z * (a.z > 0 ? k : 0.01f * k), d.w * (a.w > 0 ? k : 0.01f * k));
+    __shared__ float4 part[4 * 64];
+    rvsa_win_addend<1>(dsamp, w, avg, g, C, N, blockIdx.x, blockIdx.y, ds, part);
 }
 
 extern "C" int mtp_rvsa_sampling_bwd_win(const float* dsamp, const float* w, const float* avg, float* g, int64_t windows, int64_t C, int64_t N, mtp_stream_t stream) {
diff --git a/mtp_amd/csrc/layernorm.hip b/mtp_amd/csrc/layernorm.hip
--- a/mtp_amd/csrc/layernorm.hip
+++ b/mtp_amd/csrc/layernorm.hip
@@ -55,17 +55,28 @@
 
 struct LnWin { int Hp, Wp, pad_t, pad_l, nh, nw; };
 
-template <typename Tact, typename Tx, typename Tdx, bool GELU, int MV>
+__device__ __forceinline__ float4 as_stored(float4 v, const float*) { return v; }
+__device__ __forceinline__ float4 as_stored(float4 v, const bf16_t*) {
+    const uint32_t lo = pack_bf16x2(v.x, v.y), hi = pack_bf16x2(v.z, v.w);
+    return make_float4(bf16_bits_to_f32(lo & 0xffffu), bf16_bits_to_f32(lo >> 16), bf16_bits_to_f32(hi & 0xffffu), bf16_bits_to_f32(hi >> 16));
+}
+
+template <typename Tact, typename Tx, typename Tdx, bool GELU, int MV, bool DXSUM = false>
 __global__ __launch_bounds__(LN_THREADS) void ln_bwd_kernel(const Tact* __restrict__ dy, const Tx* __restrict__ x, const float* __restrict__ mean,
                                                            const float* __restrict__ rstd, const float* __restrict__ gamma, const float* __restrict__ beta,
                                                            const float* __restrict__ dres, const float* __restrict__ extra, Tdx* __restrict__ dx,
                                                            Tact* __restrict__ dx_copy, const float* __restrict__ copy_scale, int rows_per_sample,
                                                            float* __restrict__ dgamma_part, float* __restrict__ dbeta_part, int64_t part_ld, int64_t rows, int C,
-                                                           const float* __restrict__ win_add, LnWin wg) {
-    __shared__ float4 red[2][3][64 * MV];
+                                                           const float* __restrict__ win_add, LnWin wg, float* __restrict__ dxsum_part) {
+    __shared__ float4 red[DXSUM ? 3 : 2][3][64 * MV];
     const int lane = threadIdx.x & 63, wave = threadIdx.x >> 6;
     const int nv = C >> 2;
     float4 gacc[MV], bacc[MV], g[MV], bt[MV];
+    float4 sacc[DXSUM ? MV : 1];
+    if (DXSUM) {
+#pragma unroll
+        for (int i = 0; i < (DXSUM ? MV : 1); ++i) sacc[i] = make_float4(0, 0, 0, 0);
+    }
     int col[MV];
     bool ok[MV];
 #pragma unroll
@@ -135,6 +146,10 @@
                                          (d[i].z - xh[i].z * c1 - c2) * rs + rr[i].z + ee[i].z, (d[i].w - xh[i].w * c1 - c2) * rs + rr[i].w + ee[i].w);
             if (ok[i]) {
                 store4(dx + row * C + col[i], o);
+                if (DXSUM) {
+                    const float4 r = as_stored(o, dx);
+                    sacc[DXSUM ? i : 0].x += r.x; sacc[DXSUM ? i : 0].y += r.y; sacc[DXSUM ? i : 0].z += r.z; sacc[DXSUM ? i : 0].w += r.w;
+                }
                 if (dx_copy) store4(dx_copy + row * C + col[i], make_float4(o.x * cs, o.y * cs, o.z * cs, o.w * cs));
             }
         }
@@ -144,6 +159,7 @@
         for (int i = 0; i < MV; ++i) {
             red[0][wave - 1][lane + 64 * i] = gacc[i];
             red[1][wave - 1][lane + 64 * i] = bacc[i];
+            if (DXSUM) red[DXSUM ? 2 : 0][wave - 1][lane + 64 * i] = sacc[DXSUM ? i : 0];
         }
     }
     __syncthreads();
@@ -160,6 +176,15 @@
                 }
                 *reinterpret_cast<float4*>(dgamma_part + (int64_t)blockIdx.x * part_ld + col[i]) = a;
                 *reinterpret_cast<float4*>(dbeta_part + (int64_t)blockIdx.x * part_ld + col[i]) = b;
+                if (DXSUM) {
+                    float4 c = sacc[DXSUM ? i : 0];
+#pragma unroll
+                    for (int w = 0; w < 3; ++w) {
+                        const float4 rc = red[DXSUM ? 2 : 0][w][lane + 64 * i];
+                        c.x += rc.x; c.y += rc.y; c.z += rc.z; c.w += rc.w;
+                    }
+                    *reinterpret_cast<float4*>(dxsum_part + (int64_t)blockIdx.x * part_ld + col[i]) = c;
+                }
             }
         }
     }
@@ -435,18 +460,19 @@
     return mtp_launch_status();
 }
 
-template <typename Tact, typename Tx, typename Tdx>
+template <typename Tact, typename Tx, typename Tdx, bool DXSUM = false>
 int launch_ln_bwd(const void* dy, const void* x, const float* mean, const float* rstd, const float* gamma, const float* beta, int gelu,
                   const float* dres, const float* extra, void* dx, void* dx_copy, const float* copy_scale, int64_t rps,
-                  float* dgp, float* dbp, int64_t part_ld, int64_t rows, int64_t C, hipStream_t s, const float* win_add = nullptr, LnWin wg = LnWin{1, 1, 0, 0, 1, 1}) {
+                  float* dgp, float* dbp, int64_t part_ld, int64_t rows, int64_t C, hipStream_t s, const float* win_add = nullptr, LnWin wg = LnWin{1, 1, 0, 0, 1, 1},
+                  float* dsp = nullptr) {
     dim3 grid((unsigned)mtp_layernorm_bwd_partial_rows(rows)), block(LN_THREADS);
 #define MTP_CALL(MV_)                                                                                                                                        \
     if (gelu)                                                                                                                                                \
-        hipLaunchKernelGGL((ln_bwd_kernel<Tact, Tx, Tdx, true, MV_>), grid, block, 0, s, (const Tact*)dy, (const Tx*)x, mean, rstd, gamma, beta, dres, extra, \
-                           (Tdx*)dx, (Tact*)dx_copy, copy_scale, (int)(rps > 0 ? rps : 1), dgp, dbp, part_ld, rows, (int)C, win_add, wg);                    \
+        hipLaunchKernelGGL((ln_bwd_kernel<Tact, Tx, Tdx, true, MV_, DXSUM>), grid, block, 0, s, (const Tact*)dy, (const Tx*)x, mean, rstd, gamma, beta, dres, extra, \
+                           (Tdx*)dx, (Tact*)dx_copy, copy_scale, (int)(rps > 0 ? rps : 1), dgp, dbp, part_ld, rows, (int)C, win_add, wg, dsp);               \
     else                                                                                                                                                     \
-        hipLaunchKernelGGL((ln_bwd_kernel<Tact, Tx, Tdx, false, MV_>), grid, block, 0, s, (const Tact*)dy, (const Tx*)x, mean, rstd, gamma, beta, dres, extra, \
-                           (Tdx*)dx, (Tact*)dx_copy, copy_scale, (int)(rps > 0 ? rps : 1), dgp, dbp, part_ld, rows, (int)C, win_add, wg)
+        hipLaunchKernelGGL((ln_bwd_kernel<Tact, Tx, Tdx, false, MV_, DXSUM>), grid, block, 0, s, (const Tact*)dy, (const Tx*)x, mean, rstd, gamma, beta, dres, extra, \
+                           (Tdx*)dx, (Tact*)dx_copy, copy_scale, (int)(rps > 0 ? rps : 1), dgp, dbp, part_ld, rows, (int)C, win_add, wg, dsp)
     MTP_LN_MV(C, MTP_CALL);
 #undef MTP_CALL
     return mtp_launch_status();
@@ -532,6 +558,24 @@
     return MTP_ERR_UNSUPPORTED;
 }
 
+extern "C" int mtp_layernorm_bwd_dxsum(const void* dy, int dy_dtype, const void* x, int x_dtype, const float* mean, const float* rstd,
+                                       const float* gamma, const float* beta, int fuse_gelu, const float* dres, const float* extra, void* dx, int dx_dtype,
+                                       void* dx_copy, int copy_dtype, const float* copy_scale, int64_t rows_per_sample,
+                                       float* dgamma_part, float* dbeta_part, float* dxsum_part, int64_t part_ld, int64_t rows, int64_t C, mtp_stream_t stream) {
+    if (part_ld == 0) part_ld = C;
+    if (part_ld < C || (part_ld % 4)) return MTP_ERR_ARG;
+    if (!dy || !x || !mean || !rstd || !gamma || !dx || !dgamma_part || !dbeta_part || !dxsum_part || rows <= 0 || rows > INT32_MAX || (C % 4) || C > 256 * MAXV) return MTP_ERR_ARG;
+    if (fuse_gelu && !beta) return MTP_ERR_ARG;
+    if (dx_copy && copy_dtype != dy_dtype) return MTP_ERR_ARG;
+    if (dy_dtype == MTP_BF16 && x_dtype == MTP_BF16 && dx_dtype == MTP_BF16)
+        return launch_ln_bwd<bf16_t, bf16_t, bf16_t, true>(dy, x, mean, rstd, gamma, beta, fuse_gelu, dres, extra, dx, dx_copy, copy_scale, rows_per_sample, dgamma_part, dbeta_part,
+                                                           part_ld, rows, C, (hipStream_t)stream, nullptr, LnWin{1, 1, 0, 0, 1, 1}, dxsum_part);
+    if (dy_dtype == MTP_F32 && x_dtype == MTP_F32 && dx_dtype == MTP_F32)
+        return launch_ln_bwd<float, float, float, true>(dy, x, mean, rstd, gamma, beta, fuse_gelu, dres, extra, dx, dx_copy, copy_scale, rows_per_sample, dgamma_part, dbeta_part,
+                                                        part_ld, rows, C, (hipStream_t)stream, nullptr, LnWin{1, 1, 0, 0, 1, 1}, dxsum_part);
+    return MTP_ERR_UNSUPPORTED;
+}
+
 extern "C" int mtp_layernorm_bwd_win(const void* dy, int dy_dtype, const void* x, int x_dtype, const float* mean, const float* rstd,
                                      const float* gamma, const float* dres, const float* extra, void* dx, int dx_dtype,
                                      void* dx_copy, int copy_dtype, const float* copy_scale, int64_t rows_per_sample,
diff --git a/mtp_amd/engine.py b/mtp_amd/engine.py
--- a/mtp_amd/engine.py
+++ b/mtp_amd/engine.py
@@ -101,10 +101,6 @@
     wgrad_max_jobs = 8
     wgrad_keep = 2
 
-    @staticmethod
-    def _colsum(dy, out):
-        return ops.colsum(dy, out, accumulate=True)
-
     def _ln_bwd(self, *args, **kw):
         return ops.layernorm_bwd(*args, accumulate=True, defer=self._ln_parts, **kw)
 
@@ -191,15 +187,17 @@
                norm_ok=not ls)
         do = ops.gemm_nt(dx1_act, b.wprojT, self._e(T, C))
         dqkv = self._e(T, 3 * C)
+        win_add = None
         if b.window:
             nh, nw = ops.rvsa_windows(Hp, Wp)
             R = B * nh * nw
             H = self.heads
             dsamp = self._e(R, 5 * H, dtype=F32)
+            win_add = self._e(*s["avg"].shape, dtype=F32)
             ops.rvsa_attn_bwd(s["qkv"], s["samp"], s["o"], do, s["lse"], dqkv, dsamp,
                               P[pre + "attn.rel_pos_h"], P[pre + "attn.rel_pos_w"], P[pre + "attn.relative_position_bias_table"],
                               G[pre + "attn.rel_pos_h"], G[pre + "attn.rel_pos_w"], G[pre + "attn.relative_position_bias_table"],
-                              B, Hp, Wp, H, self.scale, accumulate=True, defer=self._ln_parts)
+                              B, Hp, Wp, H, self.scale, accumulate=True, defer=self._ln_parts, win=(b.wsamp, s["avg"], win_add))
             names = ("sampling_offsets", "sampling_scales", "sampling_angles")
             self._sl_jobs.append((s["pooled"], dsamp, [G[pre + "attn.%s.2.weight" % n].view(-1, C) for n in names],
                                   [G[pre + "attn.%s.2.bias" % n] for n in names]))
@@ -212,9 +210,6 @@
             ops.full_attn_bwd(s["qkv"], s["o"], do, s["lse"], dqkv, rel_h, rel_w, drel_h, drel_w, B, Hp, Wp, self.heads, self.scale,
                               accumulate=True, defer=self._ln_parts)
         wq.add(dqkv, s["ln1"], G[pre + "attn.qkv.weight"], G[pre + "attn.qkv.bias"])
-        win_add = None
-        if b.window:
-            win_add = ops.rvsa_sampling_bwd_win(dsamp, b.wsamp, s["avg"], self._e(*s["avg"].shape, dtype=F32))
         dln1 = ops.gemm_nt(dqkv, b.wqkvT, self._e(T, C))
         dx0, dx0_act = self._e(T, C, dtype=F32), self._e(T, C)
         self._ln_bwd(dln1, s["x"], s["mean1"], s["rstd1"], P[pre + "norm1.weight"], dx0, G[pre + "norm1.weight"], G[pre + "norm1.bias"],
@@ -338,9 +333,8 @@
         if fctx.get("p8"):
             H2, W2, H4, W4 = Hp // 2, Wp // 2, Hp // 4, Wp // 4
             if dfeats[0] is not None:
-                dz = ops.nchw_to_tokens(as_in(dfeats[0]), self._e(4 * T, C), B, Hp, Wp, 1)
+                dz = ops.nchw_to_tokens(as_in(dfeats[0]), self._e(4 * T, C), B, Hp, Wp, 1, colsum=G["fpn1.0.bias"])
                 self._convt_wgrad(dz.view(T, 4 * C), fctx["t0"], G["fpn1.0.weight"])
-                self._colsum(dz, G["fpn1.0.bias"])
                 out[0] = ops.gemm_nt(dz.view(T, 4 * C), self._fpn["fpn1.0"][1], self._e(T, C, dtype=F32))
             if dfeats[1] is not None:
                 out[1] = ops.nchw_to_tokens(as_in(dfeats[1]), self._e(T, C, dtype=F32), B, Hp, Wp, 0)
@@ -354,20 +348,17 @@
             return out
 
         if dfeats[0] is not None:
-            dy2 = ops.nchw_to_tokens(as_in(dfeats[0]), self._e(16 * T, C), B, Hp, Wp, 2)
+            dy2 = ops.nchw_to_tokens(as_in(dfeats[0]), self._e(16 * T, C), B, Hp, Wp, 2, colsum=G["fpn1.3.bias"])
             self._convt_wgrad(dy2.view(4 * T, 4 * C), fctx["g1"], G["fpn1.3.weight"])
-            self._colsum(dy2, G["fpn1.3.bias"])
             dg1 = ops.gemm_nt(dy2.view(4 * T, 4 * C), self._fpn["fpn1.3"][1], self._e(4 * T, C))
             dy1 = self._e(4 * T, C)
             self._ln_bwd(dg1, fctx["y1"].view(4 * T, C), fctx["mean"], fctx["rstd"], P["fpn1.1.ln.weight"], dy1,
-                              G["fpn1.1.ln.weight"], G["fpn1.1.ln.bias"], beta=P["fpn1.1.ln.bias"], gelu=True)
+                              G["fpn1.1.ln.weight"], G["fpn1.1.ln.bias"], beta=P["fpn1.1.ln.bias"], gelu=True, dx_colsum=G["fpn1.0.bias"])
             self._convt_wgrad(dy1.view(T, 4 * C), fctx["t0"], G["fpn1.0.weight"])
-            self._colsum(dy1, G["fpn1.0.bias"])
             out[0] = ops.gemm_nt(dy1.view(T, 4 * C), self._fpn["fpn1.0"][1], self._e(T, C, dtype=F32))
         if dfeats[1] is not None:
-            dz = ops.nchw_to_tokens(as_in(dfeats[1]), self._e(4 * T, C), B, Hp, Wp, 1)
+            dz = ops.nchw_to_tokens(as_in(dfeats[1]), self._e(4 * T, C), B, Hp, Wp, 1, colsum=G["fpn2.0.bias"])
             self._convt_wgrad(dz.view(T, 4 * C), fctx["t1"], G["fpn2.0.weight"])
-            self._colsum(dz, G["fpn2.0.bias"])
             out[1] = ops.gemm_nt(dz.view(T, 4 * C), self._fpn["fpn2.0"][1], self._e(T, C, dtype=F32))
         if dfeats[2] is not None:
             out[2] = ops.nchw_to_tokens(as_in(dfeats[2]), self._e(T, C, dtype=F32), B, Hp, Wp, 0)
diff --git a/mtp_amd/ops.py b/mtp_amd/ops.py
--- a/mtp_amd/ops.py
+++ b/mtp_amd/ops.py
@@ -294,10 +294,25 @@
 
 
 def layernorm_bwd(dy, x, mean, rstd, gamma, dx, dgamma, dbeta, beta=None, gelu=False, dres=None, extra=None,
-                  dx_copy=None, copy_scale=None, rows_per_sample=0, accumulate=False, defer=None, win_add=None, grid=None):
+                  dx_copy=None, copy_scale=None, rows_per_sample=0, accumulate=False, defer=None, win_add=None, grid=None, dx_colsum=None):
     rows, Cc = x.shape
     nblk = lib().mtp_layernorm_bwd_partial_rows(rows)
-    part = _scratch((nblk, 2 * Cc), x.device, torch.float32)
+    ncol = 3 if dx_colsum is not None else 2
+    part = _scratch((nblk, ncol * Cc), x.device, torch.float32)
+    if dx_colsum is not None:
+        assert win_add is None and dx_colsum.numel() == Cc
+        check(lib().mtp_layernorm_bwd_dxsum(_p(dy), _dt(dy), _p(x), _dt(x), _f32(mean), _f32(rstd), _f32(gamma), _f32(beta), int(gelu),
+                                            _f32(dres), _f32(extra), _p(dx), _dt(dx), _p(dx_copy), (_dt(dx_copy) if dx_copy is not None else 0),
+                                            _f32(copy_scale), rows_per_sample, part.data_ptr(), part.data_ptr() + 4 * Cc, part.data_ptr() + 8 * Cc, 3 * Cc, rows, Cc, _s()),
+              "mtp_layernorm_bwd_dxsum")
+        pair, dxs = part[:, :2 * Cc], part[:, 2 * Cc:]
+        if defer is not None and _adjacent(dgamma, dbeta) and dgamma.numel() == Cc:
+            defer.append((pair, dgamma, accumulate))
+            defer.append((dxs, dx_colsum, True))
+        else:
+            _reduce_pair(pair, Cc, dgamma, dbeta, accumulate)
+            reduce_rows(dxs, dx_colsum, True)
+        return dx
     if win_add is not None:
         B, Hp, Wp = grid
         nh, nw = rvsa_windows(Hp, Wp)
@@ -553,8 +568,12 @@
     return out
 
 
-def nchw_to_tokens(f, out, B, Hp, Wp, levels):
+def nchw_to_tokens(f, out, B, Hp, Wp, levels, colsum=None):
     Cc = f.shape[1]
+    if colsum is not None:
+        assert colsum.numel() == Cc
+        check(lib().mtp_nchw_to_tokens_colsum(_p(f), _dt(f), _p(out), _dt(out), B, Hp, Wp, Cc, levels, _f32(colsum), _s()), "mtp_nchw_to_tokens_colsum")
+        return out
     check(lib().mtp_nchw_to_tokens(_p(f), _dt(f), _p(out), _dt(out), B, Hp, Wp, Cc, levels, _s()), "mtp_nchw_to_tokens")
     return out
 
@@ -700,7 +719,8 @@
     return o, lse
 
 
-def rvsa_attn_bwd(qkv, samp, o, dout, lse, dqkv, dsamp, rel_h, rel_w, table, drel_h, drel_w, dtable, B, Hp, Wp, heads, scale, accumulate=False, defer=None):
+def rvsa_attn_bwd(qkv, samp, o, dout, lse, dqkv, dsamp, rel_h, rel_w, table, drel_h, drel_w, dtable, B, Hp, Wp, heads, scale, accumulate=False, defer=None,
+                  win=None):
     hd = qkv.shape[1] // (3 * heads)
     T, C3 = qkv.shape
     Cc = C3 // 3
@@ -710,8 +730,15 @@
     dkv = _scratch((T, 2 * Cc), dev, torch.float32)
     rel_part = _scratch((nblk, 26 * hd), dev, torch.float32)
     tab_part = _scratch((B * nh * nw, heads * 169), dev, torch.float32)
-    check(lib().mtp_rvsa_attn_bwd(_p(qkv), _f32(samp), _p(o), _p(dout), _f32(lse), _p(dqkv), _p(dkv), _f32(dsamp), _p(rel_part), _p(tab_part),
-                                  _dt(qkv), _f32(rel_h), _f32(rel_w), _f32(table), B, Hp, Wp, heads, hd, scale, _s()), "mtp_rvsa_attn_bwd")
+    if win is not None:
+        wsamp, avg, g = win
+        assert tuple(wsamp.shape) == (5 * heads, Cc) and tuple(avg.shape) == tuple(g.shape) == (B * nh * nw, Cc)
+        check(lib().mtp_rvsa_attn_bwd_win(_p(qkv), _f32(samp), _p(o), _p(dout), _f32(lse), _p(dqkv), _p(dkv), _f32(dsamp), _p(rel_part), _p(tab_part),
+                                          _dt(qkv), _f32(rel_h), _f32(rel_w), _f32(table), B, Hp, Wp, heads, hd, scale, _f32(wsamp), _f32(avg), _f32(g), _s()),
+              "mtp_rvsa_attn_bwd_win")
+    else:
+        check(lib().mtp_rvsa_attn_bwd(_p(qkv), _f32(samp), _p(o), _p(dout), _f32(lse), _p(dqkv), _p(dkv), _f32(dsamp), _p(rel_part), _p(tab_part),
+                                      _dt(qkv), _f32(rel_h), _f32(rel_w), _f32(table), B, Hp, Wp, heads, hd, scale, _s()), "mtp_rvsa_attn_bwd")
     if defer is not None and _adjacent(drel_h, drel_w) and drel_h.numel() == 13 * hd:
         defer.append((rel_part, drel_h, accumulate))
         defer.append((tab_part, dtable, accumulate, (heads, 169)))
```

Measured after the change: 1895 images/sec, median of 6. Within noise of the previous version (+0.6%).
